# Advanced-Vision-and-Learning-Lab/sparse-view-3dgs-pack

Hardware: AMD Instinct MI355X
Metric: train-step views/s (fwd+bwd) @1M Gaussians 1080p (higher is better)
Workload: dtype f32

## Files before the change

include/gsplat.h:

```cpp
#ifndef GSPLAT_H_INCLUDED
#define GSPLAT_H_INCLUDED

#include <stddef.h>
#include <stdint.h>

#ifdef __cplusplus
extern "C" {
#endif

#define GS_ABI_VERSION 7

#define GS_OK 0
#define GS_E_NULL (-1)
#define GS_E_SHAPE (-2)
#define GS_E_SCRATCH (-3)
#define GS_E_OVERFLOW (-4)
#define GS_E_UNSUPPORTED (-5)

#define GS_TILE_X 16
#define GS_TILE_Y 16
#define GS_NUM_CHANNELS 3

typedef struct GsView {
  int32_t image_height;
  int32_t image_width;
  float tanfovx;
  float tanfovy;
  float scale_modifier;
  int32_t sh_degree;
  int32_t prefiltered;
  int32_t antialiasing;
  int32_t debug;
  int32_t tile_cull;
  const float* bg;
  const float* viewmatrix;
  const float* projmatrix;
  const float* campos;
} GsView;

typedef struct GsGaussians {
  int32_t P;
  int32_t M;
  const float* means3D;
  const float* shs;
  const float* colors_precomp;
  const float* opacities;
  const float* scales;
  const float* rotations;
  const float* cov3D_precomp;
  const float* extra_channel;
  int32_t raw_activations;
  const float* extra_gain;
  const float* shs_rest;
} GsGaussians;

typedef struct GsScratch {
  void* geom;
  size_t geom_bytes;
  void* img;
  size_t img_bytes;
  void* binning;
  size_t binning_bytes;
  int64_t binning_capacity;
  const uint32_t* tile_order_hint;
  const float* tile_depth_limit;
  uint32_t* tile_order_out;
  float* tile_depth_limit_out;
  int32_t binned;
  int32_t defer_tile_order;
  const uint32_t* step_tag;
  const float* tile_depth_limit_slack;
  uint32_t* status_host;
} GsScratch;

typedef struct GsGrads {
  float* dL_dmeans3D;
  float* dL_dmeans2D;
  float* dL_dsh;
  float* dL_dcolors;
  float* dL_dopacity;
  float* dL_dscales;
  float* dL_drotations;
  float* dL_dcov3D;
  float* dL_dextra;
} GsGrads;

int gs_abi_version(void);
const char* gs_build_info(void);
size_t gs_struct_bytes(int32_t which);

int gs_scratch_bytes(int32_t P, int32_t W, int32_t H, int64_t R_capacity, size_t out[3],
                     size_t* backward_workspace_bytes);

int gs_forward_geometry(const GsView* view, const GsGaussians* g, GsScratch* scratch,
                        int32_t* radii, int32_t* num_rendered_host, void* stream);

int gs_forward_render(const GsView* view, const GsGaussians* g, GsScratch* scratch,
                      float* out_color, float* out_invdepth, void* stream);

int gs_forward_bin(const GsView* view, const GsGaussians* g, GsScratch* scratch, uint32_t* status_host, void* stream);

int gs_forward_render_x(const GsView* view, const GsGaussians* g, GsScratch* scratch,
                        float* out_color, float* out_invdepth, float* out_extra, void* stream);

int gs_backward(const GsView* view, const GsGaussians* g, const int32_t* radii,
                const GsScratch* scratch, int64_t num_rendered, const float* dL_dcolor,
                const float* dL_dinvdepth, const GsGrads* grads, void* workspace,
                size_t workspace_bytes, void* stream);

int gs_backward_x(const GsView* view, const GsGaussians* g, const int32_t* radii,
                  const GsScratch* scratch, int64_t num_rendered, const float* dL_dcolor,
                  const float* dL_dinvdepth, const float* dL_dextra_img, const GsGrads* grads,
                  void* workspace, size_t workspace_bytes, void* stream);

int gs_backward_split(const GsView* view, const GsGaussians* g, const int32_t* radii,
                      const GsScratch* scratch, int64_t num_rendered, const float* dL_dcolor,
                      const float* dL_dinvdepth, const GsGrads* grads, float* dL_dsh_rest, void* workspace,
                      size_t workspace_bytes, void* stream);

int gs_forward_render_fsgs(const GsView* view, const GsGaussians* g, GsScratch* scratch,
                           float* out_color, float* out_depth, float* out_alpha, void* stream);
int gs_backward_fsgs(const GsView* view, const GsGaussians* g, const int32_t* radii,
                     const GsScratch* scratch, int64_t num_rendered, const float* dL_dcolor,
                     const float* dL_ddepth, const float* dL_dalpha, const GsGrads* grads,
                     void* workspace, size_t workspace_bytes, void* stream);

int gs_depth_forward(const GsView* view, const GsGaussians* g, GsScratch* scratch, float* out_depth,
                     float* out_alpha, void* stream);
int gs_depth_backward(const GsView* view, const GsGaussians* g, const int32_t* radii,
                      const GsScratch* scratch, int64_t num_rendered, const float* dL_ddepth,
                      const float* dL_dalpha, int grad_flags, float* dL_dmeans3D, float* dL_dmeans2D,
                      float* dL_dopacity, void* workspace, size_t workspace_bytes, void* stream);

#define GS_DEPTH_STEP_ROWS_GIVEN 1
int gs_depth_backward_step(const GsView* view, const GsGaussians* g, const int32_t* radii,
                           const GsScratch* scratch, int64_t num_rendered, const float* dL_ddepth,
                           const float* dL_dalpha, int which, float* param, float* exp_avg, float* exp_avg_sq,
                           float lr, int32_t step, float beta1, float beta2, float eps, int32_t flags,
                           void* workspace, size_t workspace_bytes, void* stream);

int gs_mark_visible(int32_t P, const float* means3D, const float* viewmatrix,
                    const float* projmatrix, uint8_t* present, void* stream);

int gs_region_coop(int32_t form);

int gs_export_geom(const GsScratch* scratch, int32_t P, float* depths, float* means2D ,
                   float* cov3D , float* conic_opacity , float* rgb ,
                   uint8_t* clamped , uint32_t* tiles_touched, uint32_t* point_offsets,
                   void* stream);
int gs_export_binning(const GsScratch* scratch, int64_t num_rendered, uint64_t* keys_sorted,
                      uint32_t* point_list, void* stream);
int gs_export_img(const GsScratch* scratch, int32_t W, int32_t H, float* final_T,
                  uint32_t* n_contrib, uint32_t* ranges , void* stream);

typedef struct GsStepState {
  float* xyz;
  float* features;
  float* opacity;
  float* scaling;
  float* rotation;
  float* m[5];
  float* v[5];
  float lr[6];
  int32_t step[5];
  float beta1, beta2, eps;
  float* max_radii2D;
  float* xyz_gradient_accum;
  float* denom;
  const float* coef_dev;
  const double* rows_override;
  float* grad_out[5];
  float* fail_flag;
  int32_t phase;
  int32_t rows_clean;
  void* phase1_done;
  float* extra;
  float* extra_m;
  float* extra_v;
  float* gain;
  float* gain_m;
  float* gain_v;
  float lr_extra, lr_gain;
  int32_t step_extra, step_gain;
  float* grad_out_extra;
  float* grad_out_gain;
  uint8_t* grad_mask;
  uint8_t* dormant;
  int32_t sparse;
  int32_t reached_split;
  float* grad_out_rest;
} GsStepState;
#define GS_STEP_BLOCK 256
int gs_backward_step(const GsView* view, const GsGaussians* g, const int32_t* radii,
                     const GsScratch* scratch, int64_t num_rendered, const float* dL_dcolor,
                     const float* dL_dinvdepth, const GsStepState* st, void* workspace,
                     size_t workspace_bytes, void* stream);
int gs_backward_step_x(const GsView* view, const GsGaussians* g, const int32_t* radii,
                       const GsScratch* scratch, int64_t num_rendered, const float* dL_dcolor,
                       const float* dL_dinvdepth, const float* dL_dextra_img, const GsStepState* st,
                       void* workspace, size_t workspace_bytes, void* stream);
int gs_backward_step_fsgs(const GsView* view, const GsGaussians* g, const int32_t* radii,
                          const GsScratch* scratch, int64_t num_rendered, const float* dL_dcolor,
                          const float* dL_ddepth, const float* dL_dalpha, const GsStepState* st,
                          void* workspace, size_t workspace_bytes, void* stream);

int gs_step_uninstanced(const GsView* view, const GsGaussians* g, const int32_t* radii,
                        const GsScratch* scratch, const GsStepState* st, void* stream);

int gs_backward_from_rows(const GsView* view, const GsGaussians* g, const int32_t* radii,
                          const GsScratch* scratch, const double* rows, int32_t depth_mode,
                          const GsGrads* grads, void* workspace, size_t workspace_bytes, void* stream);

int gs_export_tile_order(const GsScratch* scratch, int32_t W, int32_t H, uint32_t* out, void* stream);

size_t gs_tile_depth_limit_floats(int32_t W, int32_t H);
int gs_export_tile_stop_depth(const GsScratch* scratch, int32_t W, int32_t H, float* out, void* stream);
#define GS_STATUS_CHECK(tag, num_rendered, overflow, trunc_failed) \
  ((((uint32_t)(tag)) * 2654435761u) ^ (((uint32_t)(num_rendered)) * 40503u) ^ (((uint32_t)(overflow)) << 30) ^ \
   (((uint32_t)(trunc_failed)) << 31) ^ 0x5bd1e995u)
int gs_forward_status(const GsScratch* scratch, uint32_t* out , void* stream);
int gs_forward_tile_order(const GsView* view, const GsScratch* scratch, void* stream);
int gs_debug_blend_stats(const GsScratch* scratch, int32_t P, int32_t W, int32_t H, uint64_t* out, void* stream);
int gs_export_binning_region(const GsScratch* scratch, int32_t W, int32_t H, int64_t num_rendered, uint64_t* keys_sorted,
                             uint32_t* point_list, void* stream);
size_t gs_debug_sort_tmp_bytes(int64_t n_bound);
int gs_debug_sort_pairs(const uint32_t* keys, const uint32_t* vals, const uint32_t* n_dev, int64_t n_bound, int32_t end_bit,
                        int32_t start_buf, int32_t digit_bits, int32_t depth_form, void* tmp, size_t tmp_bytes,
                        uint32_t* keys_out, uint32_t* vals_out, uint32_t* n_kept, uint32_t* digit_totals, void* stream);
int gs_debug_scan_sums(uint32_t* sums, int32_t nb, void* stream);

size_t gs_knn_tmp_bytes(int32_t P);
int gs_knn_mean_dist2(const float* xyz , int32_t P, float* out , void* tmp,
                      size_t tmp_bytes, void* stream);
int gs_knn_mean_dist2_idx(const float* xyz , int32_t P, float* out ,
                          int32_t* nearest , void* tmp, size_t tmp_bytes, void* stream);

size_t gs_grid_encode_tmp_bytes(int64_t B, int32_t D, int32_t L, int32_t C, int64_t n_slots);
int gs_grid_encode_fwd(const float* inputs, int64_t B, int32_t D, const float* embeddings, int64_t n_slots, int32_t C,
                       const int32_t* offsets, int32_t L, float S, int32_t H, int32_t gridtype, int32_t align_corners,
                       int32_t interp, float* outputs, float* dy_dx, void* stream);
int gs_grid_encode_bwd(const float* grad, const float* inputs, int64_t B, int32_t D, int64_t n_slots, int32_t C,
                       const int32_t* offsets, int32_t L, float S, int32_t H, int32_t gridtype, int32_t align_corners,
                       int32_t interp, const float* dy_dx, float* grad_embeddings, float* grad_inputs, void* tmp,
                       size_t tmp_bytes, void* stream);
int gs_sh_encode_fwd(const float* inputs, int64_t B, int32_t degree, float* outputs, void* stream);
int gs_sh_encode_bwd(const float* grad, const float* inputs, int64_t B, int32_t degree, float* grad_inputs, void* stream);

#define GS_DN_GLOBAL 1
#define GS_DN_L1 2
size_t gs_depth_norm_tmp_bytes(int32_t H, int32_t W, int32_t p_local, int32_t p_global);
int gs_depth_norm_fwd(const float* input, const float* target, int32_t H, int32_t W, int32_t p, float margin, int32_t flags,
                      void* tmp, float* loss_out, uint8_t* mask_out , void* stream);
int gs_depth_norm_bwd(const float* input, const float* target, int32_t H, int32_t W, int32_t p, float margin, int32_t flags,
                      const void* tmp, const float* dloss_dev, float* grad_input , void* stream);
int gs_depth_smooth_fwd(const float* depth, const float* img, int32_t C, int32_t H, int32_t W, void* tmp, float* loss_out,
                        void* stream);
int gs_depth_smooth_bwd(const float* depth, const float* img, int32_t C, int32_t H, int32_t W, const void* tmp,
                        const float* dloss_dev, float* grad_depth , void* stream);
int gs_dng_depth_reg_fwd(const float* input, const float* target, int32_t H, int32_t W, int32_t p_local, int32_t p_global,
                         float margin, float w_local, float w_global, float w_smooth, void* tmp, float* loss_out ,
                         uint8_t* mask_local, uint8_t* mask_global, void* stream);
int gs_dng_depth_reg_bwd(const float* input, const float* target, int32_t H, int32_t W, int32_t p_local, int32_t p_global,
                         float margin, float w_local, float w_global, float w_smooth, const void* tmp, const float* dloss_dev,
                         float* grad_input , void* stream);

#define GS_PEARSON_ID 0
#define GS_PEARSON_NEG 1
#define GS_PEARSON_RECIP200 2
#define GS_PEARSON_WRT_R 1
#define GS_PEARSON_BLOCK_ELEMS 4096
#define GS_PEARSON_MAX_BLOCKS 512
size_t gs_pearson_tmp_bytes(int64_t n);
int gs_pearson_fwd(const float* x, const float* t, int64_t n, int32_t form_a, int32_t form_b , void* tmp,
                   float* out , int32_t* branch_out, void* stream);
int gs_pearson_bwd(const float* x, const float* t, int64_t n, int32_t form_a, int32_t form_b, int32_t flags, const void* tmp,
                   const float* dout_dev, float* grad_x , float* grad_t , void* stream);

#define GS_DNG_ENC_X 32
#define GS_DNG_ENC_D 16
#define GS_DNG_HIDDEN 64
#define GS_DNG_GEO 64
#define GS_DNG_HEADS_TILE_ROWS 128
#define GS_DNG_HEADS_MAX_BLOCKS 256
size_t gs_dng_heads_tmp_bytes(int64_t B);
int gs_dng_heads_fwd(const float* enc_x, const float* enc_d, int64_t B, const float* w_s0, const float* w_s1, const float* w_s2,
                     const float* w_c0, const float* w_c1, float* sigma , float* color , int32_t max_blocks,
                     void* stream);
int gs_dng_heads_bwd(const float* enc_x, const float* enc_d, int64_t B, const float* w_s0, const float* w_s1, const float* w_s2,
                     const float* w_c0, const float* w_c1, const float* g_sigma, const float* g_color, float* g_enc_x,
                     float* g_enc_d, float* g_w_s0, float* g_w_s1, float* g_w_s2, float* g_w_c0, float* g_w_c1, void* tmp,
// ... 339 lines not shown
```

sparse-view-3dgs-pack_amd/csrc/gs_api.hip:

```cpp
#include <stdio.h>
#include <stdlib.h>
#include <string.h>
#include <math.h>

#include "gs_common.h"
#include "gs_tilecull.h"
#include "gs_prof.h"

static int check_args(const GsView* v, const GsGaussians* g) {
  if (!v || !g) return GS_E_NULL;
  if (g->P < 0 || v->image_width <= 0 || v->image_height <= 0) return GS_E_SHAPE;
  if (g->P == 0) return GS_OK;
  if (!g->means3D || !g->opacities || !v->viewmatrix || !v->projmatrix || !v->bg) return GS_E_NULL;
  if ((g->shs == nullptr) == (g->colors_precomp == nullptr)) return GS_E_SHAPE;
  const bool has_sr = g->scales != nullptr && g->rotations != nullptr;
  const bool any_sr = g->scales != nullptr || g->rotations != nullptr;
  if ((!has_sr && g->cov3D_precomp == nullptr) || (any_sr && g->cov3D_precomp != nullptr)) return GS_E_SHAPE;
  if (g->shs && (g->M < (v->sh_degree + 1) * (v->sh_degree + 1) || !v->campos)) return GS_E_SHAPE;
  if (v->sh_degree < 0 || v->sh_degree > 3) return GS_E_SHAPE;
  if (g->shs_rest && (!g->shs || g->M < 2)) return GS_E_SHAPE;
  if (v->image_width > 65535 * TILE_X || v->image_height > 65535 * TILE_Y) return GS_E_UNSUPPORTED;
  return GS_OK;
}

static bool reached_marking() {
  static const bool on = [] { const char* e = getenv("GS_REACHED_SPLIT"); return !(e && atoi(e) == 0); }();
  return on;
}
static inline bool step_uses_reached(const GsStepState* st) {
  return st && st->reached_split && !st->rows_override && !st->grad_out[0];
}

static inline void tile_grid(const GsView* v, int& gx, int& gy) {
  gx = (v->image_width + TILE_X - 1) / TILE_X;
  gy = (v->image_height + TILE_Y - 1) / TILE_Y;
}

struct RegionLayout {
  uint32_t* count;
  uint2* bucket;
  uint32_t* point_list;
  uint32_t cap;
  int rg_x, rg_y;
};
static int region_layout(const GsView* v, const GsScratch* sc, RegionLayout& rl) {
  int gx, gy;
  tile_grid(v, gx, gy);
  const size_t T = (size_t)gx * gy, N = (size_t)v->image_width * v->image_height;
  if (!sc->img || !sc->binning) return GS_E_NULL;
  if (sc->img_bytes < img_bytes(N, T)) return GS_E_SCRATCH;
  const int64_t cap = sc->binning_capacity;
  if (cap <= 0 || cap > 0xFFFFFFFFll) return GS_E_SHAPE;
  if (sc->binning_bytes < bin_bytes((size_t)cap, T)) return GS_E_SCRATCH;
  rl.rg_x = (gx + RG_TILES - 1) / RG_TILES;
  rl.rg_y = (gy + RG_TILES - 1) / RG_TILES;
  rl.cap = region_capacity(cap, rl.rg_x * rl.rg_y);
  if (rl.cap == 0) return GS_E_SHAPE;
  ImgView iv = img_view(sc->img, N, T);
  SortBufs bv = sort_view(sc->binning, (size_t)cap);
  rl.count = iv.region_count;
  rl.bucket = reinterpret_cast<uint2*>(bv.keys[0]);
  rl.point_list = bv.vals[0];
  return GS_OK;
}

extern "C" {

int gs_abi_version(void) { return GS_ABI_VERSION; }

size_t gs_struct_bytes(int32_t which) {
  switch (which) {
    case 0: return sizeof(GsView);
    case 1: return sizeof(GsGaussians);
    case 2: return sizeof(GsScratch);
    case 3: return sizeof(GsGrads);
    case 4: return sizeof(GsStepState);
    case 5: return sizeof(GsLgdwtParams);
    case 6: return sizeof(GsAdamSeg);
    default: return 0;
  }
}

const char* gs_build_info(void) {
  return "libgsplat_hip gfx950 | hipcc " __VERSION__
         " | preprocess/knn: -ffp-contract=off, blend: fast contract | radix 8-bit LSD | tile 16x16, wave64 8x8 quadrants";
}

int gs_scratch_bytes(int32_t P, int32_t W, int32_t H, int64_t R_capacity, size_t out[3], size_t* bwd_ws) {
  if (!out) return GS_E_NULL;
  if (P < 0 || W <= 0 || H <= 0 || R_capacity < 0) return GS_E_SHAPE;
  const size_t T = (size_t)((W + TILE_X - 1) / TILE_X) * ((H + TILE_Y - 1) / TILE_Y);
  out[0] = geom_bytes((size_t)P);
  out[1] = img_bytes((size_t)W * H, T);
  out[2] = bin_bytes((size_t)R_capacity, T);
  if (bwd_ws) *bwd_ws = bwd_workspace_bytes((size_t)P);
  return GS_OK;
}

int gs_forward_geometry(const GsView* v, const GsGaussians* g, GsScratch* sc, int32_t* radii,
                        int32_t* num_rendered_host, void* stream) {
  int rc = check_args(v, g);
  if (rc) return rc;
  if (!sc || !sc->geom) return GS_E_NULL;
  sc->binned = 0;
  hipStream_t s = (hipStream_t)stream;
  const int P = g->P;
  if (sc->geom_bytes < geom_bytes((size_t)P)) return GS_E_SCRATCH;
  GeomView gv = geom_view(sc->geom, (size_t)P);
  if (P == 0) {
    GS_HIP_CHECK(hipMemsetAsync(gv.hdr, 0, sizeof(GeomHeader), s));
    if (num_rendered_host) GS_HIP_CHECK(hipMemcpyAsync(num_rendered_host, &gv.hdr->num_rendered, 4, hipMemcpyDeviceToHost, s));
    return GS_OK;
  }
  if (!radii) return GS_E_NULL;
  PreprocessArgs a;
  a.P = P;
  a.D = v->sh_degree;
  a.M = g->M;
  a.means3D = g->means3D;
  a.scales = g->scales;
  a.scale_modifier = v->scale_modifier;
  a.rotations = g->rotations;
  a.opacities = g->opacities;
  a.raw_activations = g->raw_activations;
  a.shs = g->shs;
  a.shs_rest = g->shs_rest;
  a.cov3D_precomp = g->cov3D_precomp;
  a.colors_precomp = g->colors_precomp;
  a.viewmatrix = v->viewmatrix;
  a.projmatrix = v->projmatrix;
  a.campos = v->campos;
  a.W = v->image_width;
  a.H = v->image_height;
  a.focal_y = v->image_height / (2.0f * v->tanfovy);
  a.focal_x = v->image_width / (2.0f * v->tanfovx);
  a.tan_fovx = v->tanfovx;
  a.tan_fovy = v->tanfovy;
  a.radii = radii;
  tile_grid(v, a.grid_x, a.grid_y);
  a.antialiasing = v->antialiasing;
  a.extra_channel = g->extra_channel;
  a.extra_gain = g->extra_gain;
  a.tile_cull = v->tile_cull;
  a.tile_depth_limit = v->tile_cull ? sc->tile_depth_limit : nullptr;
  a.region_count = nullptr;
  a.region_bucket = nullptr;
  a.region_cap = 0;
  a.rg_x = a.rg_y = 0;
  if (v->tile_cull == 2) {
    RegionLayout rl;
    rc = region_layout(v, sc, rl);
    if (rc) return rc;
    a.region_count = rl.count;
    a.region_bucket = rl.bucket;
    a.region_cap = rl.cap;
    a.rg_x = rl.rg_x;
    a.rg_y = rl.rg_y;
    launch_region_prepare(gv, rl.count, rl.rg_x * rl.rg_y, (uint32_t)P, s);
    GS_LAUNCH_CHECK(s, v->debug);
  }
  {
    GS_PROF(ST_PREPROCESS_FWD, s);
    launch_preprocess_fwd(a, gv, s);
  }
  GS_LAUNCH_CHECK(s, v->debug);
  if (v->tile_cull != 2) {
    GS_PROF(ST_SCAN, s);
    launch_scan_block_sums(gv, P, s);
  }
  GS_LAUNCH_CHECK(s, v->debug);
  if (num_rendered_host)
    GS_HIP_CHECK(hipMemcpyAsync(num_rendered_host, &gv.hdr->num_rendered, 4, hipMemcpyDeviceToHost, s));
  return GS_OK;
}

int gs_forward_render(const GsView* v, const GsGaussians* g, GsScratch* sc, float* out_color, float* out_invdepth,
                      void* stream) {
  return gs_forward_render_x(v, g, sc, out_color, out_invdepth, nullptr, stream);
}

static int forward_bin_stage(const GsView* v, const GsScratch* sc, const GeomView& gv, const ImgView& iv, const SortBufs& bv, int P,
                             int gx, int gy, hipStream_t s) {
  int rc;
  const int64_t cap = sc->binning_capacity;
  const size_t T = (size_t)gx * gy;
  if (v->tile_cull == 2) {
    RegionLayout rl;
    rc = region_layout(v, sc, rl);
    if (rc) return rc;
    GS_PROF(ST_SORT, s);
    rc = launch_region_bin(gv, rl.count, rl.bucket, rl.cap, rl.rg_x, rl.rg_y, gx, gy, sc->tile_depth_limit, iv.ranges, rl.point_list,
                           cap, s);
    if (rc) return rc;
    GS_LAUNCH_CHECK(s, v->debug);
    return GS_OK;
  }
  launch_bin_prepare(gv, cap, iv.ranges, (int)T, s);
  GS_LAUNCH_CHECK(s, v->debug);
  if (cap > 0) {
    {
      GS_PROF(ST_SORT_DEPTH, s);
      rc = launch_radix_sort(gv.gsort, &gv.hdr->P, P, 32, 0, gv.depth_keys, s, v->debug, &gv.hdr->n_ordered);
      if (rc) return rc;
    }
    const TileBinView tb = tilebin_view((char*)sc->binning + sort_bytes((size_t)cap), (size_t)cap, T);
    rc = launch_tile_binning(gv, bv, tb, P, cap, gx, gy, v->tile_cull, sc->tile_depth_limit, iv.ranges, (v->debug & 2) ? 1 : 0, s,
                             v->debug & 1);
    if (rc) return rc;
  }
  GS_LAUNCH_CHECK(s, v->debug);
  return GS_OK;
}

static int forward_render_impl(const GsView* v, const GsGaussians* g, GsScratch* sc, float* out_color, float* out_invdepth,
                               float* out_extra, int fsgs, void* stream);

int gs_forward_bin(const GsView* v, const GsGaussians* g, GsScratch* sc, uint32_t* status_host, void* stream) {
  int rc = check_args(v, g);
  if (rc) return rc;
  if (!sc || !sc->geom || !sc->img) return GS_E_NULL;
  hipStream_t s = (hipStream_t)stream;
  const int P = g->P, W = v->image_width, H = v->image_height;
  int gx, gy;
  tile_grid(v, gx, gy);
  const size_t T = (size_t)gx * gy, N = (size_t)W * H;
  if (sc->img_bytes < img_bytes(N, T)) return GS_E_SCRATCH;
  if (P > 0) {
    if (sc->geom_bytes < geom_bytes((size_t)P)) return GS_E_SCRATCH;
    const int64_t cap = sc->binning_capacity;
    if (cap < 0) return GS_E_SHAPE;
    if (cap > 0 && (!sc->binning || sc->binning_bytes < bin_bytes((size_t)cap, T))) return GS_E_SCRATCH;
    if (cap > 0xFFFFFFFFll) return GS_E_UNSUPPORTED;
    GeomView gv = geom_view(sc->geom, (size_t)P);
    ImgView iv = img_view(sc->img, N, T);
    SortBufs bv = sort_view(sc->binning, (size_t)cap);
    rc = forward_bin_stage(v, sc, gv, iv, bv, P, gx, gy, s);
    if (rc) return rc;
  }
  sc->binned = 1;
  if (status_host) GS_HIP_CHECK(hipMemcpyAsync(status_host, sc->geom, 16, hipMemcpyDeviceToHost, s));
  return GS_OK;
}

int gs_forward_render_x(const GsView* v, const GsGaussians* g, GsScratch* sc, float* out_color, float* out_invdepth,
                        float* out_extra, void* stream) {
  if (out_extra && g && !g->extra_channel) return GS_E_NULL;
  return forward_render_impl(v, g, sc, out_color, out_invdepth, out_extra, 0, stream);
}

int gs_forward_render_fsgs(const GsView* v, const GsGaussians* g, GsScratch* sc, float* out_color, float* out_depth,
                           float* out_alpha, void* stream) {
  if (!out_depth || !out_alpha) return GS_E_NULL;
  if (v && v->antialiasing) return GS_E_UNSUPPORTED;
  return forward_render_impl(v, g, sc, out_color, out_depth, out_alpha, 1, stream);
}
// ... 771 lines not shown
```

sparse-view-3dgs-pack_amd/csrc/gs_common.h:

```cpp
#pragma once
#include <hip/hip_runtime.h>
#include <stdint.h>

#include "../../include/gsplat.h"

#define GS_BLOCK 256
#define TILE_X GS_TILE_X
#define TILE_Y GS_TILE_Y

struct GeomHeader {
  uint32_t num_rendered;
  uint32_t overflow;
  uint32_t trunc_failed;
  uint32_t zero;
  uint32_t P;
  uint32_t sort_n;
  uint32_t n_ordered;
  uint32_t region_mode;
  uint32_t step_tag;
  uint32_t pad[55];
};
#define HDR_SIDE_CURSOR 1
#define HDR_LIMITED 2
#define HDR_REACHED 3
// ... 138 lines not shown
  v.region_ranges = (uint2*)p; p += gs_align(8 * T);
  v.chunk_first = (uint32_t*)p; p += gs_align(4 * (T + 1));
  v.chunk_desc = (uint4*)p; p += gs_align(16 * mc);
  v.chunk_counts = (uint32_t*)p; p += gs_align(64 * mc);
  v.tile_start = (uint32_t*)p;
  v.max_chunks = (uint32_t)mc;
  return v;
}
static inline __host__ __device__ size_t bin_bytes(size_t cap, size_t T) { return sort_bytes(cap) + tilebin_bytes(cap, T); }

enum { GR_MX = 0, GR_MY, GR_CXX, GR_CXY, GR_CYY, GR_OP, GR_CR, GR_CG, GR_CB, GR_ID, GR_EXTRA, GR_N, GR_STRIDE = 16 };
typedef double gs_row_t;
#define GR_ROW_BYTES (GR_STRIDE * sizeof(gs_row_t))
enum { GC_MX = 0, GC_MY, GC_DMX, GC_DMY, GC_DMZ, GC_DOP, GC_C0, GC_R = GC_C0 + 7, GC_G, GC_B, GC_EXTRA, GC_STRIDE = 20 };
#define GC_REC_BYTES (GC_STRIDE * sizeof(float))
static inline __host__ __device__ size_t bwd_workspace_bytes(size_t P) {
  return gs_align(P * GR_ROW_BYTES) + gs_align(P * GC_REC_BYTES) + gs_align(4 * ((P + GS_BLOCK - 1) / GS_BLOCK + 4));
}

static inline uint32_t gs_higher_msb(uint32_t n) {
  uint32_t msb = sizeof(n) * 4;
  uint32_t step = msb;
  while (step > 1) {
    step /= 2;
    if (n >> msb)
      msb += step;
    else
      msb -= step;
  }
  if (n >> msb) msb++;
  return msb;
}

#define GS_HIP_CHECK(expr)                 \
  do {                                     \
    hipError_t _e = (expr);                \
    if (_e != hipSuccess) return (int)_e;  \
  } while (0)

static inline int gs_after_launch(hipStream_t s, int debug) {
  hipError_t e = hipGetLastError();
  if (e != hipSuccess) return (int)e;
  if (debug) {
    e = hipStreamSynchronize(s);
    if (e != hipSuccess) return (int)e;
  }
  return 0;
}
#define GS_LAUNCH_CHECK(stream, debug)             \
  do {                                             \
    int _rc = gs_after_launch((stream), (debug));  \
    if (_rc) return _rc;                           \
  } while (0)

struct PreprocessArgs {
  int P, D, M;
  const float* means3D;
  const float* scales;
  float scale_modifier;
  const float* rotations;
  const float* opacities;
  const float* shs;
  const float* shs_rest;
  const float* cov3D_precomp;
  const float* colors_precomp;
  const float* viewmatrix;
  const float* projmatrix;
  const float* campos;
  int W, H;
  float focal_x, focal_y, tan_fovx, tan_fovy;
  int* radii;
  int grid_x, grid_y;
  int antialiasing;
  const float* extra_channel;
  const float* extra_gain;
  int tile_cull;
  const float* tile_depth_limit;
  int raw_activations;
  uint32_t* region_count;
  uint2* region_bucket;
  uint32_t region_cap;
  int rg_x, rg_y;
};
int launch_preprocess_fwd(const PreprocessArgs& a, const GeomView& g, hipStream_t s);
int launch_scan_block_sums(const GeomView& g, int P, hipStream_t s);
int launch_mark_visible(int P, const float* means3D, const float* viewmatrix, uint8_t* present, hipStream_t s);

int launch_bin_prepare(const GeomView& g, int64_t capacity, uint2* ranges, int T, hipStream_t s);
int launch_radix_sort(const SortBufs& b, const uint32_t* n_dev, int64_t n_host_bound, int end_bit, int start_buf,
                      const uint32_t* first_keys, hipStream_t s, int debug, uint32_t* n_kept = nullptr, int digit_bits = 8);
int launch_scan_sums(uint32_t* sums, int nb, hipStream_t s);
int launch_tile_binning(const GeomView& g, const SortBufs& bv, const TileBinView& tb, int P, int64_t capacity, int grid_x, int grid_y,
                        int tile_cull, const float* tile_depth_limit, uint2* ranges, int force_rowwise, hipStream_t s, int debug);

#define RG_TILES 4
#define RG_MAX_ENTRIES 16384
static inline __host__ __device__ uint32_t region_capacity(int64_t capacity, int regions) {
  const int64_t c = regions > 0 ? capacity / regions : 0;
  return (uint32_t)(c > RG_MAX_ENTRIES ? RG_MAX_ENTRIES : (c < 0 ? 0 : c));
}
int launch_region_prepare(const GeomView& g, uint32_t* region_count, int regions, uint32_t P, hipStream_t s);
int launch_region_bin(const GeomView& g, const uint32_t* region_count, const uint2* region_bucket, uint32_t region_cap, int rg_x,
                      int rg_y, int grid_x, int grid_y, const float* tile_depth_limit, uint2* ranges, uint32_t* point_list,
                      int64_t capacity, hipStream_t s);
int launch_export_keys_region(const uint2* ranges, const uint32_t* point_list, const Splat* splat, int T, uint64_t* keys_sorted,
                              hipStream_t s);


int launch_render_fwd_wave(const uint2* ranges, const uint32_t* point_list, int W, int H, int grid_x, int grid_y,
                           const Splat* splat, const float* bg, float* final_T, uint32_t* n_contrib, uint32_t* tile_work,
                           const uint32_t* order_hint, const float* depth_limit, float* stop_depth, uint32_t* trunc_failed,
                           float* out_color, float* out_invdepth, float* out_extra, int fsgs, int cull, hipStream_t s,
                           uint8_t* reached = nullptr, uint32_t* reached_flag = nullptr);
int launch_export_stop_depth(const float* stop_depth, float* out, int grid_x, int grid_y, hipStream_t s);
int launch_tile_order(const uint32_t* tile_work, uint32_t* tile_order, int T, uint32_t* order_out, const float* stop_depth,
                      float* limit_out, int grid_x, int grid_y, const GeomHeader* hdr, hipStream_t s,
                      const float* slack_dev = nullptr, uint32_t* status_host = nullptr, const uint32_t* step_tag = nullptr);
int launch_zero_rows(gs_row_t* rows, size_t P, const uint32_t* tiles_touched, hipStream_t s);
int launch_render_bwd_wave(const uint2* ranges, const uint32_t* point_list, int W, int H, int grid_x, int grid_y,
                           const Splat* splat, const float* bg, const float* final_T, const uint32_t* n_contrib,
                           const uint32_t* tile_work, const uint32_t* tile_order, const float* dL_dpix,
                           const float* dL_dinvdepth, const float* dL_dextra, gs_row_t* grad_rows, int fsgs, hipStream_t s);

int launch_depth_fwd(const uint2* ranges, const uint32_t* point_list, int W, int H, int grid_x, int grid_y, const Splat* splat,
                     float* final_T, uint32_t* n_contrib, uint32_t* tile_work, float* stop_depth, float* out_depth,
                     float* out_alpha, int cull, hipStream_t s);
int launch_depth_bwd(const uint2* ranges, const uint32_t* point_list, int W, int H, int grid_x, int grid_y, const Splat* splat,
                     const float* final_T, const uint32_t* n_contrib, const uint32_t* tile_work, const uint32_t* tile_order,
                     const float* dL_ddepth, const float* dL_dalpha, gs_row_t* grad_rows, int grad_flags, hipStream_t s);
struct DepthPointArgs {
  int P;
  const float* means3D;
  const int* radii;
  const float* scales;
  const float* rotations;
  float scale_modifier;
  const float* cov3D;
  const float* viewmatrix;
  const float* projmatrix;
  float focal_x, focal_y, tan_fovx, tan_fovy;
  int skip_uninstanced;
  const uint32_t* tiles_touched;
  const gs_row_t* grad_rows;
  float* dL_dmeans3D;
  float* dL_dmeans2D;
  float* dL_dopacity;
};
int launch_depth_point_bwd(const DepthPointArgs& a, int grad_flags, hipStream_t s);
struct DepthStepArgs {
  float* param;
  float* exp_avg;
  float* exp_avg_sq;
  const float* activated;
  float lr_bc1, inv_sqrt_bc2, b1, b2, eps;
};
int launch_depth_point_step(const DepthPointArgs& a, const DepthStepArgs& st, int which, hipStream_t s);

int launch_blend_stats(const uint2* ranges, const uint32_t* point_list, int W, int H, int grid_x, int grid_y, const Splat* splat,
                       const uint32_t* n_contrib, const uint32_t* tile_work, unsigned long long* out, hipStream_t s);

struct PreprocessBwdArgs {
  int P, D, M;
  const float* means3D;
  const int* radii;
  const float* shs;
  const float* shs_rest;
  const float* scales;
  const float* rotations;
  const float* opacities;
  const float* colors_precomp;
  float scale_modifier;
  const float* cov3D;
  const float* viewmatrix;
  const float* projmatrix;
  const float* campos;
  float focal_x, focal_y, tan_fovx, tan_fovy;
  int antialiasing;
  int has_invdepth;
  int has_extra;
  const float* extra_raw;
  const float* extra_gain;
  float* gain_partials;
  int raw_activations;
  int skip_uninstanced;
// ... 29 lines not shown
```

sparse-view-3dgs-pack_amd/csrc/gs_preprocess.hip:

```cpp
#include "gs_common.h"
#include "gs_tilecull.h"
#include "gs_math.h"

template <typename SH>
GS_DEV V3 color_from_sh(int deg, V3 pos, V3 campos, const SH& sh, uint32_t& clamped) {
  V3 dir = pos - campos;
  dir = dir / length3(dir);
  V3 result = SH_C0 * sh(0);
  if (deg > 0) {
    float x = dir.x, y = dir.y, z = dir.z;
    result = result - SH_C1 * y * sh(1) + SH_C1 * z * sh(2) - SH_C1 * x * sh(3);
    if (deg > 1) {
      float xx = x * x, yy = y * y, zz = z * z;
      float xy = x * y, yz = y * z, xz = x * z;
      result = result + SH_C2_0 * xy * sh(4) + SH_C2_1 * yz * sh(5) + SH_C2_2 * (2.0f * zz - xx - yy) * sh(6) +
               SH_C2_3 * xz * sh(7) + SH_C2_4 * (xx - yy) * sh(8);
      if (deg > 2) {
        result = result + SH_C3_0 * y * (3.0f * xx - yy) * sh(9) + SH_C3_1 * xy * z * sh(10) +
                 SH_C3_2 * y * (4.0f * zz - xx - yy) * sh(11) + SH_C3_3 * z * (2.0f * zz - 3.0f * xx - 3.0f * yy) * sh(12) +
                 SH_C3_4 * x * (4.0f * zz - xx - yy) * sh(13) + SH_C3_5 * z * (xx - yy) * sh(14) +
                 SH_C3_6 * x * (xx - 3.0f * yy) * sh(15);
      }
    }
  }
  result.x += 0.5f;
  result.y += 0.5f;
  result.z += 0.5f;
  clamped = (result.x < 0 ? 1u : 0u) | (result.y < 0 ? 2u : 0u) | (result.z < 0 ? 4u : 0u);
  return {fmaxf(result.x, 0.0f), fmaxf(result.y, 0.0f), fmaxf(result.z, 0.0f)};
}

struct ShRegs {
  float f[48];
  __device__ __forceinline__ V3 operator()(int k) const { return {f[3 * k], f[3 * k + 1], f[3 * k + 2]}; }
};
struct ShMem {
  const float* p;
  __device__ __forceinline__ V3 operator()(int k) const { return {p[3 * k], p[3 * k + 1], p[3 * k + 2]}; }
};
struct ShMemSplit {
  const float *dc, *rest;
  __device__ __forceinline__ V3 operator()(int k) const {
    const float* p = k == 0 ? dc : rest + 3 * (k - 1);
    return {p[0], p[1], p[2]};
  }
};

#ifndef GS_LIMIT_TILES_IN_LDS
#define GS_LIMIT_TILES_IN_LDS 0
#endif
#define GS_LIMIT_LDS_MAX_FLOATS (GS_LIMIT_TILES_IN_LDS ? 10240 : 4096)
extern __shared__ float s_limit[];
static inline size_t preprocess_limit_lds_floats(const PreprocessArgs& a) {
  if (!a.tile_depth_limit) return 0;
  const size_t T = (size_t)a.grid_x * a.grid_y, all = depth_limit_floats((uint32_t)a.grid_x, (uint32_t)a.grid_y);
  const size_t want = GS_LIMIT_TILES_IN_LDS ? all : all - T;
  return want <= GS_LIMIT_LDS_MAX_FLOATS ? want : 0;
}

#ifndef GS_REGION_COOP_DEFAULT
#define GS_REGION_COOP_DEFAULT 1
#endif
#define GS_COOP_PAIRS 2
struct CoopWave {
  uint32_t pref[64];
  uint32_t dbits[64];
  uint32_t r0[64];
  uint32_t nrx[64];
  uint32_t tiles[64];
};

template <bool COOP>
__global__ void __launch_bounds__(GS_BLOCK) preprocess_fwd_kernel(PreprocessArgs a, GeomView g, int lds_floats) {
  const int idx = blockIdx.x * GS_BLOCK + threadIdx.x;
  uint32_t tiles = 0, entries = TB_ENTRIES_UNKNOWN;
  const int T = a.grid_x * a.grid_y;
  int p0 = 0, p1 = 0, p2 = 0, p3 = 0, n_pend = 0;
  uint32_t s0 = 0xFFFFFFFFu, s1 = 0xFFFFFFFFu, s2 = 0xFFFFFFFFu, s3 = 0xFFFFFFFFu, dbits = 0;
  auto bump = [&]() {
    if (n_pend > 0) s0 = atomicAdd(&a.region_count[(size_t)p0 * RG_COUNT_STRIDE], 1u);
    if (n_pend > 1) s1 = atomicAdd(&a.region_count[(size_t)p1 * RG_COUNT_STRIDE], 1u);
    if (n_pend > 2) s2 = atomicAdd(&a.region_count[(size_t)p2 * RG_COUNT_STRIDE], 1u);
    if (n_pend > 3) s3 = atomicAdd(&a.region_count[(size_t)p3 * RG_COUNT_STRIDE], 1u);
    n_pend = 0;
  };
  auto collect = [&]() {
    const uint2 entry = make_uint2(dbits, (uint32_t)idx);
    if (s0 < a.region_cap) a.region_bucket[(size_t)p0 * a.region_cap + s0] = entry;
    if (s1 < a.region_cap) a.region_bucket[(size_t)p1 * a.region_cap + s1] = entry;
    if (s2 < a.region_cap) a.region_bucket[(size_t)p2 * a.region_cap + s2] = entry;
    if (s3 < a.region_cap) a.region_bucket[(size_t)p3 * a.region_cap + s3] = entry;
    s0 = s1 = s2 = s3 = 0xFFFFFFFFu;
  };
  const int lidx = min(idx, a.P - 1);
  typedef const __attribute__((address_space(4))) float* GsConstFloatPtr;
  float vm[16], pm[16], cam[3];
  {
    const GsConstFloatPtr vmp = (GsConstFloatPtr)(uintptr_t)a.viewmatrix, pmp = (GsConstFloatPtr)(uintptr_t)a.projmatrix;
    const GsConstFloatPtr cp = (GsConstFloatPtr)(uintptr_t)a.campos;
#pragma unroll
    for (int k = 0; k < 16; k++) { vm[k] = vmp[k]; pm[k] = pmp[k]; }
    cam[0] = cp[0]; cam[1] = cp[1]; cam[2] = cp[2];
  }
  const bool own_cov = a.cov3D_precomp == nullptr;
  const float* sc_p = own_cov ? a.scales + 3 * (size_t)lidx : a.cov3D_precomp + 6 * (size_t)lidx;
  const float* rq_p = own_cov ? a.rotations + 4 * (size_t)lidx : a.cov3D_precomp + 6 * (size_t)lidx;
  float op_in = a.opacities[lidx];
  V3 p_orig = {a.means3D[3 * (size_t)lidx], a.means3D[3 * (size_t)lidx + 1], a.means3D[3 * (size_t)lidx + 2]};
  V3 sc_in = {sc_p[0], sc_p[1], sc_p[2]};
  V4 rq_in = {rq_p[0], rq_p[1], rq_p[2], rq_p[3]};
  if (lds_floats) {
    const float* src = a.tile_depth_limit + (GS_LIMIT_TILES_IN_LDS ? 0 : T);
    for (int i = threadIdx.x; i < lds_floats; i += GS_BLOCK) s_limit[i] = src[i];
    __syncthreads();
  }
  asm volatile("" : "+v"(op_in), "+v"(sc_in.x), "+v"(sc_in.y), "+v"(sc_in.z), "+v"(rq_in.x), "+v"(rq_in.y), "+v"(rq_in.z),
               "+v"(rq_in.w));
  const GsLdsFloatPtr lds_seg = (GsLdsFloatPtr)s_limit + (GS_LIMIT_TILES_IN_LDS ? T : 0);
  if (idx == 0) {
    g.hdr->pad[HDR_LIMITED] = a.tile_depth_limit ? 1u : 0u;
    g.hdr->pad[HDR_REACHED] = 0u;
  }
  const int segs_x = (int)depth_limit_segs_x((uint32_t)a.grid_x);
  auto region_bound = [&](int rx, int ry) {
    float bound = -__builtin_inff();
#pragma unroll
    for (int k = 0; k < RG_TILES; k++) {
      const int ty = min(ry * RG_TILES + k, a.grid_y - 1);
      const float v = lds_floats ? lds_seg[ty * segs_x + rx] : a.tile_depth_limit[(size_t)T + ty * segs_x + rx];
      bound = fmaxf(bound, v);
    }
    return bound;
  };
  Splat sp;
  sp.x = sp.y = sp.depth = sp.invdepth = 0.f;
  sp.cxx = sp.cxy = sp.cyy = sp.opacity = 0.f;
  sp.r = sp.g = sp.b = 0.f;
  sp.extra = 0.f;
  int radius_out = 0;
  sp.rect_min = sp.rect_max = sp.tiles = sp.clamped = 0;
  float cov3D[6] = {0, 0, 0, 0, 0, 0};
  bool write_cov = false;
  bool reached = false;
  uint32_t big_n = 0, big_r0 = 0, big_nrx = 0;

  auto finish = [&]() {
    sp.clamped |= (tiles ? entries : 0u) << 16;
    if (!(a.tile_depth_limit && tiles == 0)) {
      if (a.colors_precomp == nullptr) {
        V3 campos = {cam[0], cam[1], cam[2]};
        V3 rgb;
        uint32_t cl = 0;
        if (a.M == 16 && a.shs_rest) {
          ShRegs sh;
          const float* dc = a.shs + (size_t)idx * 3;
          const float* rest = a.shs_rest + (size_t)idx * 45;
          const int nfl = 3 * (a.D + 1) * (a.D + 1) - 3;
          sh.f[0] = dc[0]; sh.f[1] = dc[1]; sh.f[2] = dc[2];
#pragma unroll
          for (int k = 0; k < 45; k++) sh.f[3 + k] = k < nfl ? rest[k] : 0.f;
          bump();
          rgb = color_from_sh(a.D, p_orig, campos, sh, cl);
        } else if (a.M == 16) {
          ShRegs sh;
          const float4* src = reinterpret_cast<const float4*>(a.shs + (size_t)idx * 48);
          const int nvec = a.D == 0 ? 1 : (a.D == 1 ? 3 : (a.D == 2 ? 7 : 12));
#pragma unroll
          for (int k = 0; k < 12; k++) {
            if (k < nvec) {
              float4 v = src[k];
              sh.f[4 * k] = v.x; sh.f[4 * k + 1] = v.y; sh.f[4 * k + 2] = v.z; sh.f[4 * k + 3] = v.w;
            } else {
              sh.f[4 * k] = sh.f[4 * k + 1] = sh.f[4 * k + 2] = sh.f[4 * k + 3] = 0.f;
            }
          }
          bump();
          rgb = color_from_sh(a.D, p_orig, campos, sh, cl);
        } else if (a.shs_rest) {
          bump();
          ShMemSplit sh{a.shs + (size_t)idx * 3, a.shs_rest + (size_t)idx * (a.M - 1) * 3};
          rgb = color_from_sh(a.D, p_orig, campos, sh, cl);
        } else {
          bump();
          ShMem sh{a.shs + (size_t)idx * a.M * 3};
          rgb = color_from_sh(a.D, p_orig, campos, sh, cl);
        }
        sp.r = rgb.x; sp.g = rgb.y; sp.b = rgb.z;
        sp.clamped |= cl;
      } else {
        bump();
        sp.r = a.colors_precomp[3 * idx];
        sp.g = a.colors_precomp[3 * idx + 1];
        sp.b = a.colors_precomp[3 * idx + 2];
      }
    }
    sp.tiles = tiles;
  };

  bool write_record = true;
  auto store_record = [&](int half) {
    float4* dst = reinterpret_cast<float4*>(&g.splat[idx]);
    const float4* srcv = reinterpret_cast<const float4*>(&sp);
// ... 256 lines not shown
        coop_collect();
      }
      coop_bump(base);
    }
    if (idx < a.P) store_geometry();
    if (reached) finish();
    if (idx < a.P) {
      if (write_record) store_record(1);
      collect();
    }
  } else if (idx < a.P) {
    store_geometry();
    if (write_record) store_record(1);
    collect();
    if (a.tile_cull != 2) g.depth_keys[idx] = tiles ? __float_as_uint(sp.depth) : 0xFFFFFFFFu;
  }
  if constexpr (COOP) coop_collect();
  __shared__ uint32_t red[GS_BLOCK / 64];
  uint32_t v = tiles;
#pragma unroll
  for (int off = 32; off >= 1; off >>= 1) v += __shfl_down(v, off, 64);
  if ((threadIdx.x & 63) == 0) red[threadIdx.x >> 6] = v;
  __syncthreads();
  if (threadIdx.x == 0) g.block_sums[blockIdx.x] = red[0] + red[1] + red[2] + red[3];
}

__global__ void __launch_bounds__(1024) scan_block_sums_kernel(GeomView g, int nb, uint32_t P) {
  __shared__ uint32_t wsum[16];
  __shared__ uint32_t carry_s;
  const int tid = threadIdx.x, lane = tid & 63, wid = tid >> 6;
  if (tid == 0) carry_s = 0;
  __syncthreads();
  for (int base = 0; base < nb; base += 1024) {
    int i = base + tid;
    uint32_t v = (i < nb) ? g.block_sums[i] : 0u;
    uint32_t inc = v;
#pragma unroll
    for (int off = 1; off < 64; off <<= 1) {
      uint32_t t = __shfl_up(inc, off, 64);
      if (lane >= off) inc += t;
    }
    if (lane == 63) wsum[wid] = inc;
    __syncthreads();
    uint32_t woff = 0;
    for (int w = 0; w < wid; w++) woff += wsum[w];
    uint32_t carry = carry_s;
    if (i < nb) g.block_sums[i] = carry + woff + inc - v;
    __syncthreads();
    if (tid == 1023) carry_s = carry + woff + inc;
    __syncthreads();
  }
  if (tid == 0) {
    g.block_sums[nb] = carry_s;
    g.hdr->num_rendered = carry_s;
    g.hdr->overflow = 0;
    g.hdr->P = P;
    g.hdr->region_mode = 0;
    g.hdr->pad[HDR_SIDE_CURSOR] = 0;
  }
}

__global__ void __launch_bounds__(GS_BLOCK) mark_visible_kernel(int P, const float* means3D, const float* vm,
                                                                uint8_t* present) {
  const int idx = blockIdx.x * GS_BLOCK + threadIdx.x;
  if (idx >= P) return;
  V3 p = {means3D[3 * idx], means3D[3 * idx + 1], means3D[3 * idx + 2]};
  V3 pv = xform4x3(p, vm);
  present[idx] = !(pv.z <= 0.2f);
}

static int g_region_coop = -1;
static int region_coop_form() {
  if (g_region_coop < 0) {
    const char* e = getenv("GS_REGION_COOP");
    g_region_coop = e ? (atoi(e) != 0 ? 1 : 0) : GS_REGION_COOP_DEFAULT;
  }
  return g_region_coop;
}
extern "C" int gs_region_coop(int32_t form) {
  if (form >= 0) g_region_coop = form ? 1 : 0;
  return region_coop_form();
}

int launch_preprocess_fwd(const PreprocessArgs& a, const GeomView& g, hipStream_t s) {
  const int nb = (a.P + GS_BLOCK - 1) / GS_BLOCK;
  const size_t lds = preprocess_limit_lds_floats(a);
  const bool coop = a.tile_cull == 2 && region_coop_form() && a.rg_x <= 0xFFFF && a.rg_y <= 0xFFFF &&
                    (long long)a.rg_x * a.rg_y <= (1ll << 26);
  if (coop)
    hipLaunchKernelGGL(preprocess_fwd_kernel<true>, dim3(nb), dim3(GS_BLOCK), 4 * lds, s, a, g, (int)lds);
  else
    hipLaunchKernelGGL(preprocess_fwd_kernel<false>, dim3(nb), dim3(GS_BLOCK), 4 * lds, s, a, g, (int)lds);
  return 0;
}
int launch_scan_block_sums(const GeomView& g, int P, hipStream_t s) {
  const int nb = (P + GS_BLOCK - 1) / GS_BLOCK;
  hipLaunchKernelGGL(scan_block_sums_kernel, dim3(1), dim3(1024), 0, s, g, nb, (uint32_t)P);
  return 0;
}
int launch_mark_visible(int P, const float* means3D, const float* viewmatrix, uint8_t* present, hipStream_t s) {
  hipLaunchKernelGGL(mark_visible_kernel, dim3((P + GS_BLOCK - 1) / GS_BLOCK), dim3(GS_BLOCK), 0, s, P, means3D,
                     viewmatrix, present);
  return 0;
}
```

sparse-view-3dgs-pack_amd/csrc/gs_regionbin.hip:

```cpp
#include "gs_common.h"
#include "gs_tilecull.h"

#define RB_THREADS 1024
#define RB_WAVES (RB_THREADS / 64)
#define RB_TILES (RG_TILES * RG_TILES)

__global__ void __launch_bounds__(GS_BLOCK) region_prepare_kernel(GeomHeader* hdr, uint32_t* __restrict__ region_count,
                                                                   int regions, uint32_t P) {
  const int i = blockIdx.x * GS_BLOCK + threadIdx.x;
  if (i < regions) region_count[(size_t)i * RG_COUNT_STRIDE] = 0u;
  if (i == 0) {
    hdr->num_rendered = 0u;
    hdr->overflow = 0u;
    hdr->trunc_failed = 0u;
    hdr->zero = 0u;
    hdr->P = P;
    hdr->sort_n = 0u;
    hdr->n_ordered = 0u;
    hdr->region_mode = 1u;
    hdr->pad[HDR_SIDE_CURSOR] = 0u;
  }
}

__global__ void __launch_bounds__(RB_THREADS) region_bin_kernel(GeomHeader* hdr, const Splat* __restrict__ splat,
                                                                 const uint32_t* __restrict__ region_count,
                                                                 const uint2* __restrict__ region_bucket, uint32_t region_cap,
                                                                 int rg_x, int grid_x, int grid_y,
                                                                 const float* __restrict__ depth_limit,
                                                                 uint2* __restrict__ ranges, uint32_t* __restrict__ point_list,
                                                                 uint32_t capacity, uint32_t n_pad_max) {
  extern __shared__ unsigned long long s_key[];
  __shared__ uint32_t s_wcnt[RB_WAVES][RB_TILES];
  __shared__ uint32_t s_off[RB_TILES + 1];
  __shared__ uint32_t s_base;
  __shared__ float s_lim[RB_TILES];
  const int tid = threadIdx.x, lane = tid & 63, wid = tid >> 6;
  const int r = blockIdx.x, rx = r % rg_x, ry = r / rg_x;
  const uint32_t cnt_raw = region_count[(size_t)r * RG_COUNT_STRIDE];
  const uint32_t n = min(min(cnt_raw, region_cap), n_pad_max);
  if (tid == 0) {
    atomicMax(&hdr->zero, cnt_raw);
    if (cnt_raw > n) hdr->overflow = 1u;
  }
  if (tid < RB_TILES) {
    const int ty = ry * RG_TILES + (tid >> 2), tx = rx * RG_TILES + (tid & 3);
    s_lim[tid] = (depth_limit && ty < grid_y && tx < grid_x) ? depth_limit[ty * grid_x + tx] : __builtin_inff();
  }
  uint32_t n_pad = 64;
  while (n_pad < n) n_pad <<= 1;
  const uint2* bucket = region_bucket + (size_t)r * region_cap;
  for (uint32_t i = tid; i < n_pad; i += RB_THREADS) {
    unsigned long long k = ~0ull;
    if (i < n) {
      const uint2 e = bucket[i];
      k = ((unsigned long long)e.x << 32) | (unsigned long long)e.y;
    }
    s_key[i] = k;
  }
  __syncthreads();
  auto step = [&](uint32_t k, uint32_t j) {
    for (uint32_t i = tid; i < (n_pad >> 1); i += RB_THREADS) {
      const uint32_t lo = ((i & ~(j - 1u)) << 1) | (i & (j - 1u));
      const uint32_t hi = lo | j;
      const unsigned long long a = s_key[lo], b = s_key[hi];
      const bool up = (lo & k) == 0u;
      if ((a > b) == up) {
        s_key[lo] = b;
        s_key[hi] = a;
      }
    }
  };
  for (uint32_t k = 2; k <= n_pad; k <<= 1) {
    uint32_t j = k >> 1;
    for (; j > 64; j >>= 1) {
      step(k, j);
      __syncthreads();
    }
    for (; j > 0; j >>= 1) {
      step(k, j);
      __builtin_amdgcn_fence(__ATOMIC_RELEASE, "wavefront");
      __builtin_amdgcn_wave_barrier();
      __builtin_amdgcn_fence(__ATOMIC_ACQUIRE, "wavefront");
    }
    if (k >= 128u || k == n_pad) __syncthreads();
  }
  for (uint32_t e = tid; e < n; e += RB_THREADS) {
    const uint32_t id = (uint32_t)s_key[e];
    const float4* rec = reinterpret_cast<const float4*>(&splat[id]);
    const float4 ra = rec[0], rc = rec[1];
    const uint4 tail = reinterpret_cast<const uint4*>(rec)[3];
    const TileCull tc = tilecull_setup(1, ra.x, ra.y, rc.x, rc.y, rc.z, rc.w);
    const uint32_t rminx = tail.x & 0xFFFFu, rminy = tail.x >> 16, rmaxx = tail.y & 0xFFFFu, rmaxy = tail.y >> 16;
    uint32_t mask = 0;
#pragma unroll
// ... 13 lines not shown
    }
    s_key[e] = ((unsigned long long)mask << 32) | (unsigned long long)id;
  }
  __syncthreads();
  const uint32_t per_wave = ((n + RB_WAVES * 64 - 1) / (RB_WAVES * 64)) * 64;
  const uint32_t w_lo = min((uint32_t)wid * per_wave, n), w_hi = min(w_lo + per_wave, n);
  uint32_t my_cnt = 0;
  for (uint32_t e0 = w_lo; e0 < w_hi; e0 += 64) {
    const uint32_t e = e0 + lane;
    const uint32_t m = e < w_hi ? (uint32_t)(s_key[e] >> 32) : 0u;
#pragma unroll
    for (uint32_t t = 0; t < RB_TILES; t++) {
      const uint32_t c = (uint32_t)__popcll(__ballot((m >> t) & 1u));
      if (lane == (int)t) my_cnt += c;
    }
  }
  if (lane < RB_TILES) s_wcnt[wid][lane] = my_cnt;
  __syncthreads();
  if (tid < RB_TILES) {
    uint32_t run = 0;
#pragma unroll
    for (int w = 0; w < RB_WAVES; w++) {
      const uint32_t c = s_wcnt[w][tid];
      s_wcnt[w][tid] = run;
      run += c;
    }
    s_off[tid + 1] = run;
  }
  __syncthreads();
  if (tid == 0) {
    uint32_t run = 0;
    s_off[0] = 0;
    for (int t = 0; t < RB_TILES; t++) {
      const uint32_t c = s_off[t + 1];
      s_off[t] = run;
      run += c;
    }
    s_off[RB_TILES] = run;
    uint32_t base = 0xFFFFFFFFu;
    if (run) {
      const uint32_t at = atomicAdd(&hdr->num_rendered, run);
      if ((unsigned long long)at + run <= (unsigned long long)capacity) base = at;
      else hdr->overflow = 1u;
    } else {
      base = 0u;
    }
    s_base = base;
  }
  __syncthreads();
  const uint32_t base = s_base;
  if (tid < RB_TILES) {
    const int ty = ry * RG_TILES + (tid >> 2), tx = rx * RG_TILES + (tid & 3);
    if (ty < grid_y && tx < grid_x) {
      const uint32_t b = base + s_off[tid], c = s_off[tid + 1] - s_off[tid];
      ranges[ty * grid_x + tx] = (base == 0xFFFFFFFFu || c == 0u) ? make_uint2(0u, 0u) : make_uint2(b, b + c);
    }
  }
  if (base == 0xFFFFFFFFu) return;
  uint32_t run = 0;
  const unsigned long long lt_mask = lane == 0 ? 0ull : (~0ull >> (64 - lane));
  for (uint32_t e0 = w_lo; e0 < w_hi; e0 += 64) {
    const uint32_t e = e0 + lane;
    const unsigned long long k = e < w_hi ? s_key[e] : 0ull;
    const uint32_t m = (uint32_t)(k >> 32), id = (uint32_t)k;
#pragma unroll
    for (uint32_t t = 0; t < RB_TILES; t++) {
      const unsigned long long b = __ballot((m >> t) & 1u);
      const uint32_t before = (uint32_t)__shfl((int)run, (int)t, 64);
      if ((m >> t) & 1u) point_list[base + s_off[t] + s_wcnt[wid][t] + before + (uint32_t)__popcll(b & lt_mask)] = id;
      if (lane == (int)t) run += (uint32_t)__popcll(b);
    }
  }
}

__global__ void __launch_bounds__(GS_BLOCK) export_keys_region_kernel(const uint2* __restrict__ ranges,
                                                                      const uint32_t* __restrict__ point_list,
                                                                      const Splat* __restrict__ splat,
                                                                      uint64_t* __restrict__ keys_sorted) {
  const uint2 r = ranges[blockIdx.x];
  for (uint32_t i = r.x + threadIdx.x; i < r.y; i += GS_BLOCK)
    keys_sorted[i] = ((uint64_t)blockIdx.x << 32) | (uint64_t)__float_as_uint(splat[point_list[i]].depth);
}

int launch_region_prepare(const GeomView& g, uint32_t* region_count, int regions, uint32_t P, hipStream_t s) {
  hipLaunchKernelGGL(region_prepare_kernel, dim3((regions + GS_BLOCK - 1) / GS_BLOCK > 0 ? (regions + GS_BLOCK - 1) / GS_BLOCK : 1),
                     dim3(GS_BLOCK), 0, s, g.hdr, region_count, regions, P);
  return 0;
}

int launch_region_bin(const GeomView& g, const uint32_t* region_count, const uint2* region_bucket, uint32_t region_cap, int rg_x,
                      int rg_y, int grid_x, int grid_y, const float* tile_depth_limit, uint2* ranges, uint32_t* point_list,
                      int64_t capacity, hipStream_t s) {
  uint32_t n_pad = 1024;
  while (n_pad < region_cap && n_pad < RG_MAX_ENTRIES) n_pad <<= 1;
  const size_t lds = (size_t)n_pad * sizeof(unsigned long long);
  static_assert(RG_MAX_ENTRIES * sizeof(unsigned long long) <= 160 * 1024, "a region's sort must fit gfx950's 160 KB of LDS");
  static size_t lds_allowed[64] = {};
  int dev = 0;
  if (hipGetDevice(&dev) != hipSuccess || dev < 0 || dev >= 64) dev = -1;
  if (dev < 0 || lds > lds_allowed[dev]) {
    hipError_t e = hipFuncSetAttribute((const void*)region_bin_kernel, hipFuncAttributeMaxDynamicSharedMemorySize, (int)lds);
    if (e != hipSuccess) return (int)e;
    if (dev >= 0) lds_allowed[dev] = lds;
  }
  const uint32_t cap32 = capacity > 0xFFFFFFFFll ? 0xFFFFFFFFu : (capacity < 0 ? 0u : (uint32_t)capacity);
  hipLaunchKernelGGL(region_bin_kernel, dim3(rg_x * rg_y), dim3(RB_THREADS), lds, s, g.hdr, g.splat, region_count, region_bucket,
                     region_cap, rg_x, grid_x, grid_y, tile_depth_limit, ranges, point_list, cap32, n_pad);
  const hipError_t le = hipGetLastError();
  return le == hipSuccess ? 0 : (int)le;
}

int launch_export_keys_region(const uint2* ranges, const uint32_t* point_list, const Splat* splat, int T, uint64_t* keys_sorted,
                              hipStream_t s) {
  hipLaunchKernelGGL(export_keys_region_kernel, dim3(T), dim3(GS_BLOCK), 0, s, ranges, point_list, splat, keys_sorted);
  return 0;
}
```

sparse-view-3dgs-pack_amd/gsplat_amd/capi.py:

```python
import ctypes as C
import os

c_f_p = C.c_void_p


class GsView(C.Structure):
    _fields_ = [
        ("image_height", C.c_int32),
        ("image_width", C.c_int32),
        ("tanfovx", C.c_float),
        ("tanfovy", C.c_float),
        ("scale_modifier", C.c_float),
        ("sh_degree", C.c_int32),
        ("prefiltered", C.c_int32),
        ("antialiasing", C.c_int32),
        ("debug", C.c_int32),
        ("tile_cull", C.c_int32),
        ("bg", C.c_void_p),
        ("viewmatrix", C.c_void_p),
        ("projmatrix", C.c_void_p),
        ("campos", C.c_void_p),
    ]


class GsGaussians(C.Structure):
    _fields_ = [
        ("P", C.c_int32),
        ("M", C.c_int32),
        ("means3D", C.c_void_p),
        ("shs", C.c_void_p),
        ("colors_precomp", C.c_void_p),
        ("opacities", C.c_void_p),
        ("scales", C.c_void_p),
        ("rotations", C.c_void_p),
        ("cov3D_precomp", C.c_void_p),
        ("extra_channel", C.c_void_p),
        ("raw_activations", C.c_int32),
        ("extra_gain", C.c_void_p),
        ("shs_rest", C.c_void_p),
    ]


class GsScratch(C.Structure):
    _fields_ = [
        ("geom", C.c_void_p),
        ("geom_bytes", C.c_size_t),
        ("img", C.c_void_p),
        ("img_bytes", C.c_size_t),
        ("binning", C.c_void_p),
        ("binning_bytes", C.c_size_t),
        ("binning_capacity", C.c_int64),
        ("tile_order_hint", C.c_void_p),
        ("tile_depth_limit", C.c_void_p),
        ("tile_order_out", C.c_void_p),
        ("tile_depth_limit_out", C.c_void_p),
        ("binned", C.c_int32),
        ("defer_tile_order", C.c_int32),
        ("step_tag", C.c_void_p),
        ("tile_depth_limit_slack", C.c_void_p),
        ("status_host", C.c_void_p),
    ]


class GsGrads(C.Structure):
    _fields_ = [
        ("dL_dmeans3D", C.c_void_p),
        ("dL_dmeans2D", C.c_void_p),
        ("dL_dsh", C.c_void_p),
        ("dL_dcolors", C.c_void_p),
        ("dL_dopacity", C.c_void_p),
        ("dL_dscales", C.c_void_p),
        ("dL_drotations", C.c_void_p),
        ("dL_dcov3D", C.c_void_p),
        ("dL_dextra", C.c_void_p),
    ]


class GsLgdwtParams(C.Structure):
    _fields_ = [("lambda_dssim", C.c_float), ("n_pix", C.c_float), ("n_band1", C.c_float), ("n_band2", C.c_float),
                ("dwt_w", C.c_float * 8), ("patch_w", C.c_float * 3), ("patch_weight", C.c_float),
                ("patch_elems_per_sel", C.c_float), ("dwt_enable", C.c_int32), ("patch_enable", C.c_int32),
                ("reset_sums", C.c_int32), ("custom_base", C.c_int32), ("w_l1", C.c_float), ("w_ssim", C.c_float)]


class GsAdamSeg(C.Structure):
    _fields_ = [("begin", C.c_int64), ("end", C.c_int64), ("lr_a", C.c_float), ("lr_b", C.c_float),
                ("period", C.c_int32), ("split", C.c_int32), ("step", C.c_int32), ("row_width", C.c_int32)]


class GsAdamTensor(C.Structure):
    _fields_ = [("param", C.c_void_p), ("grad", C.c_void_p), ("exp_avg", C.c_void_p), ("exp_avg_sq", C.c_void_p),
                ("n", C.c_int64), ("row_width", C.c_int32), ("step", C.c_int32), ("lr", C.c_float), ("pad", C.c_int32)]


ADAM_NO_BIAS_CORRECTION = 1
DEPTH_STEP_ROWS_GIVEN = 1
ADAM_MAX_TENSORS = 8


class GsStepState(C.Structure):
    _fields_ = [("xyz", C.c_void_p), ("features", C.c_void_p), ("opacity", C.c_void_p), ("scaling", C.c_void_p),
                ("rotation", C.c_void_p), ("m", C.c_void_p * 5), ("v", C.c_void_p * 5), ("lr", C.c_float * 6),
                ("step", C.c_int32 * 5), ("beta1", C.c_float), ("beta2", C.c_float), ("eps", C.c_float),
                ("max_radii2D", C.c_void_p), ("xyz_gradient_accum", C.c_void_p), ("denom", C.c_void_p),
                ("coef_dev", C.c_void_p), ("rows_override", C.c_void_p), ("grad_out", C.c_void_p * 5),
                ("fail_flag", C.c_void_p), ("phase", C.c_int32), ("rows_clean", C.c_int32),
                ("phase1_done", C.c_void_p),
                ("extra", C.c_void_p), ("extra_m", C.c_void_p), ("extra_v", C.c_void_p), ("gain", C.c_void_p),
                ("gain_m", C.c_void_p), ("gain_v", C.c_void_p), ("lr_extra", C.c_float), ("lr_gain", C.c_float),
                ("step_extra", C.c_int32), ("step_gain", C.c_int32), ("grad_out_extra", C.c_void_p),
                ("grad_out_gain", C.c_void_p), ("grad_mask", C.c_void_p), ("dormant", C.c_void_p), ("sparse", C.c_int32),
                ("reached_split", C.c_int32),
                ("grad_out_rest", C.c_void_p)]


_P = C.c_void_p
_I32 = C.c_int32
_I64 = C.c_int64
_F = C.c_float
_SZ = C.c_size_t

PROTOTYPES = {
    "abi_version": (C.c_int, []),
    "struct_bytes": (C.c_size_t, [C.c_int32]),
    "build_info": (C.c_char_p, []),
    "scratch_bytes": (C.c_int, [_I32, _I32, _I32, _I64, C.POINTER(_SZ), C.POINTER(_SZ)]),
    "forward_geometry": (C.c_int, [C.POINTER(GsView), C.POINTER(GsGaussians), C.POINTER(GsScratch), _P, _P, _P]),
    "forward_render": (C.c_int, [C.POINTER(GsView), C.POINTER(GsGaussians), C.POINTER(GsScratch), _P, _P, _P]),
    "backward": (C.c_int, [C.POINTER(GsView), C.POINTER(GsGaussians), _P, C.POINTER(GsScratch), _I64, _P, _P,
                           C.POINTER(GsGrads), _P, _SZ, _P]),
    "forward_render_x": (C.c_int, [C.POINTER(GsView), C.POINTER(GsGaussians), C.POINTER(GsScratch), _P, _P, _P, _P]),
    "backward_split": (C.c_int, [C.POINTER(GsView), C.POINTER(GsGaussians), _P, C.POINTER(GsScratch), _I64, _P, _P,
                                 C.POINTER(GsGrads), _P, _P, _SZ, _P]),
    "backward_x": (C.c_int, [C.POINTER(GsView), C.POINTER(GsGaussians), _P, C.POINTER(GsScratch), _I64, _P, _P, _P,
                             C.POINTER(GsGrads), _P, _SZ, _P]),
    "forward_render_fsgs": (C.c_int, [C.POINTER(GsView), C.POINTER(GsGaussians), C.POINTER(GsScratch), _P, _P, _P, _P]),
    "backward_fsgs": (C.c_int, [C.POINTER(GsView), C.POINTER(GsGaussians), _P, C.POINTER(GsScratch), _I64, _P, _P, _P,
                                C.POINTER(GsGrads), _P, _SZ, _P]),
    "depth_forward": (C.c_int, [C.POINTER(GsView), C.POINTER(GsGaussians), C.POINTER(GsScratch), _P, _P, _P]),
    "depth_backward": (C.c_int, [C.POINTER(GsView), C.POINTER(GsGaussians), _P, C.POINTER(GsScratch), _I64, _P, _P, C.c_int,
                                 _P, _P, _P, _P, _SZ, _P]),
    "depth_backward_step": (C.c_int, [C.POINTER(GsView), C.POINTER(GsGaussians), _P, C.POINTER(GsScratch), _I64, _P, _P, C.c_int,
                                      _P, _P, _P, _F, _I32, _F, _F, _F, _I32, _P, _SZ, _P]),
    "step_uninstanced": (C.c_int, [C.POINTER(GsView), C.POINTER(GsGaussians), _P, C.POINTER(GsScratch),
                                   C.POINTER(GsStepState), _P]),
    "backward_step": (C.c_int, [C.POINTER(GsView), C.POINTER(GsGaussians), _P, C.POINTER(GsScratch), _I64, _P, _P,
                                C.POINTER(GsStepState), _P, _SZ, _P]),
    "backward_step_x": (C.c_int, [C.POINTER(GsView), C.POINTER(GsGaussians), _P, C.POINTER(GsScratch), _I64, _P, _P, _P,
                                  C.POINTER(GsStepState), _P, _SZ, _P]),
    "backward_step_fsgs": (C.c_int, [C.POINTER(GsView), C.POINTER(GsGaussians), _P, C.POINTER(GsScratch), _I64, _P, _P, _P,
                                     C.POINTER(GsStepState), _P, _SZ, _P]),
    "backward_from_rows": (C.c_int, [C.POINTER(GsView), C.POINTER(GsGaussians), _P, C.POINTER(GsScratch), _P, _I32,
                                     C.POINTER(GsGrads), _P, _SZ, _P]),
    "mark_visible": (C.c_int, [_I32, _P, _P, _P, _P, _P]),
    "region_coop": (C.c_int, [_I32]),
    "export_geom": (C.c_int, [C.POINTER(GsScratch), _I32, _P, _P, _P, _P, _P, _P, _P, _P, _P]),
    "export_binning": (C.c_int, [C.POINTER(GsScratch), _I64, _P, _P, _P]),
    "export_img": (C.c_int, [C.POINTER(GsScratch), _I32, _I32, _P, _P, _P, _P]),
    "export_tile_order": (C.c_int, [C.POINTER(GsScratch), _I32, _I32, _P, _P]),
    "export_tile_stop_depth": (C.c_int, [C.POINTER(GsScratch), _I32, _I32, _P, _P]),
    "forward_status": (C.c_int, [C.POINTER(GsScratch), _P, _P]),
    "forward_tile_order": (C.c_int, [C.POINTER(GsView), C.POINTER(GsScratch), _P]),
    "forward_bin": (C.c_int, [C.POINTER(GsView), C.POINTER(GsGaussians), C.POINTER(GsScratch), _P, _P]),
    "export_binning_region": (C.c_int, [C.POINTER(GsScratch), _I32, _I32, _I64, _P, _P, _P]),
    "debug_blend_stats": (C.c_int, [C.POINTER(GsScratch), _I32, _I32, _I32, _P, _P]),
    "debug_sort_tmp_bytes": (_SZ, [_I64]),
    "debug_sort_pairs": (C.c_int, [_P, _P, _P, _I64, _I32, _I32, _I32, _I32, _P, _SZ, _P, _P, _P, _P, _P]),
    "debug_scan_sums": (C.c_int, [_P, _I32, _P]),
    "tile_depth_limit_floats": (C.c_size_t, [_I32, _I32]),
    "knn_tmp_bytes": (_SZ, [_I32]),
    "knn_mean_dist2": (C.c_int, [_P, _I32, _P, _P, _SZ, _P]),
    "knn_mean_dist2_idx": (C.c_int, [_P, _I32, _P, _P, _P, _SZ, _P]),
    "grid_encode_tmp_bytes": (_SZ, [_I64, _I32, _I32, _I32, _I64]),
    "grid_encode_fwd": (C.c_int, [_P, _I64, _I32, _P, _I64, _I32, _P, _I32, _F, _I32, _I32, _I32, _I32, _P, _P, _P]),
    "grid_encode_bwd": (C.c_int, [_P, _P, _I64, _I32, _I64, _I32, _P, _I32, _F, _I32, _I32, _I32, _I32, _P, _P, _P, _P,
                                  _SZ, _P]),
    "sh_encode_fwd": (C.c_int, [_P, _I64, _I32, _P, _P]),
    "sh_encode_bwd": (C.c_int, [_P, _P, _I64, _I32, _P, _P]),
    "depth_norm_tmp_bytes": (_SZ, [_I32, _I32, _I32, _I32]),
    "depth_norm_fwd": (C.c_int, [_P, _P, _I32, _I32, _I32, _F, _I32, _P, _P, _P, _P]),
    "depth_norm_bwd": (C.c_int, [_P, _P, _I32, _I32, _I32, _F, _I32, _P, _P, _P, _P]),
    "depth_smooth_fwd": (C.c_int, [_P, _P, _I32, _I32, _I32, _P, _P, _P]),
    "depth_smooth_bwd": (C.c_int, [_P, _P, _I32, _I32, _I32, _P, _P, _P, _P]),
    "dng_depth_reg_fwd": (C.c_int, [_P, _P, _I32, _I32, _I32, _I32, _F, _F, _F, _F, _P, _P, _P, _P, _P]),
    "dng_depth_reg_bwd": (C.c_int, [_P, _P, _I32, _I32, _I32, _I32, _F, _F, _F, _F, _P, _P, _P, _P]),
    "pearson_tmp_bytes": (_SZ, [_I64]),
    "pearson_fwd": (C.c_int, [_P, _P, _I64, _I32, _I32, _P, _P, _P, _P]),
    "pearson_bwd": (C.c_int, [_P, _P, _I64, _I32, _I32, _I32, _P, _P, _P, _P, _P]),
    "dng_heads_tmp_bytes": (_SZ, [_I64]),
    "dng_heads_fwd": (C.c_int, [_P, _P, _I64, _P, _P, _P, _P, _P, _P, _P, _I32, _P]),
    "dng_heads_bwd": (C.c_int, [_P, _P, _I64, _P, _P, _P, _P, _P, _P, _P, _P, _P, _P, _P, _P, _P, _P, _P, _SZ, _I32, _P]),
    "dng_reg_tmp_bytes": (_SZ, [_I64]),
    "dng_reg_fwd": (C.c_int, [_P, _P, _I64, C.c_double, C.c_double, C.c_double, _I32, _I32, _P, _P, _P]),
    "dng_reg_bwd": (C.c_int, [_P, _P, _I64, _I32, _P, _P, _P, _P, _P, _P]),
    "view_dirs_fwd": (C.c_int, [_P, _P, _I64, _P, _P]),
    "view_dirs_bwd": (C.c_int, [_P, _P, _I64, _P, _P, _P]),
    "near_mask": (C.c_int, [_P, _I64, _P, _I32, _F, _P, _P]),
    "dtu_mask": (C.c_int, [_P, _I32, _I32, _F, _I32, _P, _P, _P, _P]),
    "masked_tmp_bytes": (_SZ, [_I64]),
    "masked_fill_fwd": (C.c_int, [_P, _P, _I64, _P, _P, _P, _P]),
    "masked_fill_bwd": (C.c_int, [_P, _P, _I64, _P, _P]),
    "alpha_penalty_fwd": (C.c_int, [_P, _P, _I64, _P, _P, _P]),
    "alpha_penalty_bwd": (C.c_int, [_P, _P, _I64, _P, _P, _P, _P]),
    "dng_colour_rule": (C.c_int, [_P, _P, _P, _I64, _I32, _F, _F, _I32, _I32, _F, _F, _I32, _F, _P, _P]),
    "blender_tmp_bytes": (_SZ, [_I64]),
    "blender_target": (C.c_int, [_P, _P, _I32, _I32, _F, _P, _P, _P, _P, _P]),
    "dng_white_rule": (C.c_int, [_P, _P, _P, _I64, _F, _F, _P, _P]),
    "dng_white_rule_sh": (C.c_int, [_P, _P, _P, _I32, _I32, _P, _P, _P, _I64, _F, _F, _P, _P, _P]),
    "l1_fwd": (C.c_int, [_P, _P, _I64, _P, _P]),
    "l1_bwd": (C.c_int, [_P, _P, _I64, _F, _P, _I32, _P]),
    "dwt_haar_fwd": (C.c_int, [_P, _I32, _I32, _I32, _P, _P, _P, _P, _P]),
    "dwt_haar_bwd": (C.c_int, [_P, _P, _P, _P, _I32, _I32, _I32, _P, _P]),
    "dwt2_l1_fwd": (C.c_int, [_P, _P, _I32, _I32, _I32, _P, _P]),
    "dwt2_l1_bwd": (C.c_int, [_P, _P, _I32, _I32, _I32, _P, _P, _I32, _P]),
    "elf_map": (C.c_int, [_P, _I32, _I32, _I32, _P, _P, _P]),
    "patch_means": (C.c_int, [_P, _I32, _I32, _I32, _P, _P]),
    "patch_dwt_fwd": (C.c_int, [_P, _P, _I32, _I32, _I32, _I32, _P, _P, _P]),
    "patch_dwt_bwd": (C.c_int, [_P, _P, _I32, _I32, _I32, _I32, _P, _P, _P, _I32, _P]),
    "ssim_fwd": (C.c_int, [_P, _P, _I32, _I32, _I32, _I32, _F, _F, _P, _P, _P, _P, _P]),
    "ssim_bwd": (C.c_int, [_P, _P, _I32, _I32, _I32, _I32, _F, _F, _P, _P, _P, _P, _P, _P]),
    "dwt_partials_count": (C.c_int64, [_I32, _I32, _I32]),
    "l1_dwt2_patch_fwd_clamp_p": (C.c_int, [_P, _P, _I32, _I32, _I32, _I32, _P, _P, _P, _P]),
    "l1_partials_count": (C.c_int64, [_I64]),
    "l1_fwd_p": (C.c_int, [_P, _P, _I64, _P, _P]),
    "depth_l1_partials_count": (C.c_int64, [_I64]),
    "depth_l1": (C.c_int, [_P, _P, _P, _I64, _P, _F, _P, _P, _P]),
    "lgdwt_combine_pp": (C.c_int, [_P, _P, _I64, _P, _I64, _P, _I64, _P, C.POINTER(GsLgdwtParams), _P, _P]),
    "l1_bwd_dev": (C.c_int, [_P, _P, _I64, _P, _P, _I32, _P]),
    "l1_dwt2_fwd": (C.c_int, [_P, _P, _I32, _I32, _I32, _P, _P, _P]),
    "l1_dwt2_fwd_clamp": (C.c_int, [_P, _P, _I32, _I32, _I32, _P, _P, _P, _P]),
    "l1_dwt2_patch_fwd_clamp": (C.c_int, [_P, _P, _I32, _I32, _I32, _I32, _P, _P, _P, _P, _P, _P]),
    "l1_dwt2_patch_bwd": (C.c_int, [_P, _P, _I32, _I32, _I32, _I32, _P, _P, _P, _P, _P, _I32, _P]),
    "l1_dwt2_bwd": (C.c_int, [_P, _P, _I32, _I32, _I32, _P, _P, _P, _I32, _P]),
    "ssim_fwd_sum": (C.c_int, [_P, _P, _I32, _I32, _I32, _I32, _F, _F, _P, _P, _P, _P, _P]),
    "ssim_bwd_uniform": (C.c_int, [_P, _P, _I32, _I32, _I32, _I32, _P, _P, _P, _P, _P, _I32, _P, _P]),
    "lgdwt_combine": (C.c_int, [_P, _P, C.POINTER(GsLgdwtParams), _P, _P]),
    "lgdwt_combine_p": (C.c_int, [_P, _P, _I64, _P, C.POINTER(GsLgdwtParams), _P, _P]),
    "ssim_partials_count": (C.c_int64, [_I32, _I32, _I32, _I32]),
    "ssim_fwd_partials": (C.c_int, [_P, _P, _I32, _I32, _I32, _I32, _F, _F, _P, _P, _P, _P, _P]),
    "lgdwt_fused_fwd": (C.c_int, [_P, _P, _I32, _I32, _I32, _F, _F, _I32, _P, _P, _P, _P, _P, _P, _P]),
    "lgdwt_fused_bwd": (C.c_int, [_P, _P, _I32, _I32, _I32, _I32, _I32, _P, _P, _P, _P, _P, _P, _P]),
    "adam_step": (C.c_int, [_P, _P, _P, _P, _I64, C.POINTER(GsAdamSeg), _I32, _F, _F, _F, _I32, _P]),
    "adam_step_gated": (C.c_int, [_P, _P, _P, _P, _I64, C.POINTER(GsAdamSeg), _I32, _F, _F, _F, _I32, _P, _P]),
    "adam_step_masked": (C.c_int, [_P, _P, _P, _P, _I64, C.POINTER(GsAdamSeg), _I32, _F, _F, _F, _I32, _P, _P, _P]),
    "adam_step_tensors": (C.c_int, [C.POINTER(GsAdamTensor), _I32, _I64, _F, _F, _F, _I32, _P, _P]),
    "activations_fwd": (C.c_int, [_P, _P, _P, _I32, _P, _P, _P, _P]),
    "activations_bwd": (C.c_int, [_P, _P, _P, _I32, _P, _P, _P, _P, _P, _P, _P]),
    "densify_stats": (C.c_int, [_P, _P, _I32, _P, _P, _P, _P]),
    "densify_tmp_bytes": (_SZ, [_I32]),
    "densify_plan": (C.c_int, [_P, _P, _P, _P, _I32, _I32, _F, _F, _F, _F, _F, _I32, _P, _SZ, _P]),
    "densify_emit": (C.c_int, [_P, _SZ, _P, _P, _P, _P, _I32, _I32, _I32, _I32, _I32, _I32, _I32, _P, _P, _P]),
    "morton_codes": (C.c_int, [_P, _I64, _P, _P, _P, _P]),
    "densify_gather": (C.c_int, [_P, _P, _P, _I32, _P, _P, _P, _I32, _P, _P, _P, _I32, C.POINTER(C.c_int32), _I32, _I32, _F, _P]),
    "densify_plan_gated": (C.c_int, [_P, _P, _P, _P, _I32, _I32, _F, _F, _F, _F, _F, _I32, _F, _P, _SZ, _P]),
    "prune_tmp_bytes": (_SZ, [_I32]),
    "prune_plan": (C.c_int, [_P, _I32, _P, _SZ, _P]),
    "prune_emit": (C.c_int, [_P, _SZ, _P, _P, _I32, _I32, _P, _P, _P, _P, _P, _P, _P, _P, _P]),
    "densify_fsgs_tmp_bytes": (_SZ, [_I32]),
    "densify_fsgs_plan": (C.c_int, [_P, _P, _P, _P, _P, _I32, _I32, _F, _F, _F, _F, _F, _F, _I32, _P, _SZ, _P, _P]),
    "densify_fsgs_merge": (C.c_int, [_P, _SZ, _P, _I32, _F, _I32, _P]),
    "densify_fsgs_emit": (C.c_int, [_P, _SZ, _P, _P, _P, _P, _I32, _I32, _I32, _I32, _I32, _I32, _I32, _P, _P, _P]),
    "densify_fsgs_prox_plan": (C.c_int, [_P, _SZ, _I32, _P, _I32, _P, _P, _F, _I32, _P, _SZ, _P]),
    "densify_fsgs_final": (C.c_int, [_P, _SZ, _P, _P, _P, _I32, _I32, _I32, _I32, _I32, _P, _P, _P, _P, _P, _P]),
    "densify_fsgs_gather": (C.c_int, [_P, _P, _P, _P, _I32, _P, _P, _P, _I32, _P, _P, _P, _I32, C.POINTER(C.c_int32), _I32, _I32, _I32,
                                      _I32, _F, _P]),
    "profile_enable": (C.c_int, [_I32]),
    "profile_only": (C.c_int, [_I32]),
    "profile_reset": (C.c_int, []),
    "profile_stage_count": (C.c_int, []),
    "rows_pack": (C.c_int, [_P, _I32, _I32, C.POINTER(C.c_int32), _P, _P, _I32, _P, _P]),
    "rows_unpack": (C.c_int, [_P, _I32, _I32, C.POINTER(C.c_int32), _P, _P, _I32, _P, _P]),
    "export_row_mask": (C.c_int, [C.POINTER(GsScratch), _I32, _P, _P]),
    "profile_stage_name": (C.c_char_p, [_I32]),
    "profile_read": (C.c_int, [C.POINTER(C.c_double), C.POINTER(_I64), _I32]),
    "image_stage_partials_count": (C.c_int64, [_I32, _I32]),
    "image_stage_fwd": (C.c_int, [_P, _P, _P, _I32, _I32, _P, _P]),
    "image_stage_bwd": (C.c_int, [_P, _P, _P, _P, _I32, _I32, _P, _P, _P]),
    "exposure_adam": (C.c_int, [_P, _I64, _I32, _P, _P, _P, _P, _I32, _F, C.c_double, C.c_double, _F, _I32, _P, _P]),
    "eval_partials_count": (C.c_int64, [_I32, _I32, _I32]),
    "eval_tmp_bytes": (_SZ, [_I32, _I32, _I32]),
    "eval_metrics": (C.c_int, [_P, _P, _P, _I32, _I32, _I32, _I32, _F, _F, _P, _SZ, _P, _P, _P]),
    "resize_tmp_bytes": (_SZ, [_I32, _I32, _I32, _I32, _I32]),
    "resize_bicubic_u8": (C.c_int, [_P, _I32, _I32, _I32, _I32, _I32, _P, _P, _I32, _P, _P, _I32, _P, _SZ, _P, _P, _P]),
    "eval_ssim_sk_tmp_bytes": (_SZ, [_I32, _I32, _I32]),
    "eval_ssim_sk": (C.c_int, [_P, _P, _P, _I32, _I32, _I32, _I32, _P, _SZ, _P, _P]),
    "lpips_packed_floats": (C.c_int64, [_I32, _I32]),
    "lpips_pack_weights": (C.c_int, [_P, _I32, _I32, _P, _P]),
    "lpips_tmp_bytes": (_SZ, [_I32, _I32]),
    "lpips_vgg": (C.c_int, [_P, _P, _P, _I32, _I32, _I32, _I32, _P, _P, _P, _P, _SZ, _P, _P]),
    "lpips_conv3x3_relu": (C.c_int, [_P, _P, _P, _I32, _I32, _I32, _I32, _I32, _P, _P]),
    "lpips_maxpool2": (C.c_int, [_P, _I64, _I32, _I32, _P, _P]),
    "lpips_distance_tmp_bytes": (_SZ, [_I32, _I32]),
    "lpips_distance": (C.c_int, [_P, _P, _P, _I32, _I32, _I32, _P, _SZ, _P, _P]),
    "depth_vis_tmp_bytes": (_SZ, [_I32, _I32]),
    "depth_vis": (C.c_int, [_P, _P, _I32, _I32, _I32, _P, _P, _SZ, _P, _P, _P, _P, _P]),
    "wef_tmp_bytes": (_SZ, [_I32, _I32, _I32, _I32]),
    "wef_maps": (C.c_int, [_P, _P, _I32, _I32, _I32, _I32, _P, _SZ, _P, _P, _P]),
    "wef_grid": (C.c_int, [_P, _I32, _I32, _I32, _P, _I32, _I32, _P, _P, _P]),
    "charbonnier_tmp_bytes": (_SZ, [_I64]),
    "charbonnier_fwd": (C.c_int, [_P, _P, _I64, C.c_double, _P, _SZ, _P, _P]),
    "charbonnier_bwd": (C.c_int, [_P, _P, _I64, C.c_double, _P, _P, _P, _P]),
    "depth_scales_tmp_bytes": (_SZ, [_I64]),
    "depth_scales": (C.c_int, [_P, _I64, _P, _P, _I64, _P, _P, _P, _P, _I32, _I32, _I32, _P, _SZ, _P, _P]),
    "invdepth_prepare": (C.c_int, [_P, _I32, _I32, _I32, _I32, _I32, C.c_float, _I32, C.c_float, C.c_float, C.c_float, _P, _P, _P]),
    "image_ingest_tmp_bytes": (_SZ, [_I32, _I32, _I32, _I32, _I32, _I32]),
    "image_ingest": (C.c_int, [_P, _I32, _I32, _I32, _I32, _I32, _P, _P, _I32, _P, _P, _I32, _I32, _P, _SZ, _P, _P, _P, _P]),
}

DEVICE_ONLY = ("export_row_mask", "backward_step", "backward_step_x", "backward_step_fsgs", "step_uninstanced", "export_tile_order", "export_tile_stop_depth", "forward_status", "forward_bin", "export_binning_region", "region_coop", "debug_blend_stats", "adam_step_gated", "tile_depth_limit_floats", "profile_enable", "profile_only", "profile_reset", "profile_stage_count", "profile_stage_name", "profile_read",
               "forward_render_x", "backward_x", "forward_tile_order",
               "image_stage_partials_count", "image_stage_fwd", "image_stage_bwd", "exposure_adam",
               "lgdwt_fused_fwd", "lgdwt_fused_bwd",
               "grid_encode_tmp_bytes", "grid_encode_fwd", "grid_encode_bwd", "sh_encode_fwd", "sh_encode_bwd",
               "depth_norm_tmp_bytes", "depth_norm_fwd", "depth_norm_bwd", "depth_smooth_fwd", "depth_smooth_bwd",
               "dng_depth_reg_fwd", "dng_depth_reg_bwd",
               "pearson_tmp_bytes", "pearson_fwd", "pearson_bwd",
               "dng_heads_tmp_bytes", "dng_heads_fwd", "dng_heads_bwd",
               "dng_reg_tmp_bytes", "dng_reg_fwd", "dng_reg_bwd", "view_dirs_fwd", "view_dirs_bwd", "near_mask",
               "dtu_mask", "masked_tmp_bytes", "masked_fill_fwd", "masked_fill_bwd", "alpha_penalty_fwd", "alpha_penalty_bwd",
               "dng_colour_rule",
               "blender_tmp_bytes", "blender_target", "dng_white_rule", "dng_white_rule_sh",
               "densify_tmp_bytes", "densify_plan", "densify_emit", "morton_codes", "densify_gather",
               "densify_fsgs_tmp_bytes", "densify_fsgs_plan", "densify_fsgs_merge", "densify_fsgs_emit", "densify_fsgs_prox_plan",
               "densify_fsgs_final", "densify_fsgs_gather",
               "densify_plan_gated", "prune_tmp_bytes", "prune_plan", "prune_emit",
               "eval_partials_count", "eval_tmp_bytes", "eval_metrics",
               "resize_tmp_bytes", "resize_bicubic_u8", "eval_ssim_sk_tmp_bytes", "eval_ssim_sk",
               "lpips_packed_floats", "lpips_pack_weights", "lpips_tmp_bytes", "lpips_vgg", "lpips_conv3x3_relu",
               "lpips_maxpool2", "lpips_distance_tmp_bytes", "lpips_distance",
               "depth_vis_tmp_bytes", "depth_vis",
               "wef_tmp_bytes", "wef_maps", "wef_grid", "charbonnier_tmp_bytes", "charbonnier_fwd", "charbonnier_bwd",
               "depth_scales_tmp_bytes", "depth_scales", "invdepth_prepare",
               "image_ingest_tmp_bytes", "image_ingest",
               "depth_forward", "depth_backward",
               "depth_backward_step",
               "adam_step_tensors", "backward_split",
               "debug_sort_tmp_bytes", "debug_sort_pairs", "debug_scan_sums")

ERRORS = {-1: "GS_E_NULL", -2: "GS_E_SHAPE", -3: "GS_E_SCRATCH", -4: "GS_E_OVERFLOW", -5: "GS_E_UNSUPPORTED"}


class GsError(RuntimeError):
    def __init__(self, fn, code):
        self.code = code
        what = ERRORS.get(code, "hipError_t %d" % code if code > 0 else "error %d" % code)
        super().__init__("%s failed: %s" % (fn, what))


class CApi:

    def __init__(self, path, prefix="gs_", optional=()):
        if not os.path.exists(path):
            raise ImportError(
                "gsplat native library not found at %s - build it first (python __graft_entry__.py "
                "or `make -C sparse-view-3dgs-pack_amd/csrc`); there is no fallback path." % path)
        self.path = path
        self.prefix = prefix
        self.lib = C.CDLL(path)
        self.missing = []
        for name, (res, args) in PROTOTYPES.items():
            try:
                f = getattr(self.lib, prefix + name)
            except AttributeError:
                if name in optional:
                    self.missing.append(name)
                    continue
                raise ImportError("%s does not export %s%s" % (path, prefix, name))
            f.restype = res
            f.argtypes = args
            setattr(self, "_" + name, f)

    def call(self, name, *args):
        rc = getattr(self, "_" + name)(*args)
        if rc != 0:
            raise GsError(self.prefix + name, rc)

    def raw(self, name):
        return getattr(self, "_" + name)


def read_profile(api):
    n = api.raw("profile_stage_count")()
    ms = (C.c_double * n)()
    cnt = (C.c_int64 * n)()
    api.call("profile_read", ms, cnt, n)
    return {api.raw("profile_stage_name")(i).decode(): (ms[i], cnt[i]) for i in range(n) if cnt[i] > 0}
```

sparse-view-3dgs-pack_amd/gsplat_amd/raster.py:

```python
import ctypes as C
import os

import torch

from .capi import GsGaussians, GsGrads, GsScratch, GsView

NUM_CHANNELS = 3
_DEPTH_ONLY = 2


def _ptr(t):
    if t is None or t.numel() == 0:
        return None
    return t.data_ptr()


def _prep(t, device):
    if t is None or t.numel() == 0:
        return None
    if t.dtype != torch.float32:
        t = t.float()
    if t.device != device:
        t = t.to(device)
    return t.contiguous()


def _regions(W, H):
    return ((((W + 15) // 16) + 3) // 4) * ((((H + 15) // 16) + 3) // 4)


class _Forward:
    __slots__ = ("device", "stream", "view", "g", "P", "W", "H", "geom", "img", "radii", "out_color", "out_invdepth",
                 "out_extra", "fsgs", "extra", "cache", "use_order", "use_limit", "static", "cur", "status")

    def __init__(self, device, stream, view, g, P, W, H, geom, img, radii, out_color, out_invdepth, out_extra, fsgs, extra,
                 cache, use_order, use_limit, static):
        self.device, self.stream, self.view, self.g = device, stream, view, g
        self.P, self.W, self.H = P, W, H
        self.geom, self.img, self.radii = geom, img, radii
        self.out_color, self.out_invdepth, self.out_extra = out_color, out_invdepth, out_extra
        self.fsgs, self.extra = fsgs, extra
        self.cache, self.use_order, self.use_limit, self.static = cache, use_order, use_limit, static
        self.cur = self.status = None


class _Last:
    __slots__ = ("geom", "P", "view", "g", "keep", "raw", "step", "radii", "img", "done")

    def __init__(self, geom, P, view, g, keep, raw):
        self.geom, self.P, self.view, self.g, self.keep, self.raw = geom, P, view, g, keep, raw
        self.step = self.radii = self.img = self.done = None


class RasterBackend:

    def __init__(self, api, device_type="cuda"):
        self.api = api
        self.device_type = device_type
        self._pinned = None
        self._capacity_hint = 0
        self._capacity_hint_limited = 0
        self.optimistic = os.environ.get("GS_SYNC_FORWARD", "0") != "1"
        self.tile_cull = os.environ.get("GS_TILE_CULL", "1") != "0"
        self.binning = os.environ.get("GS_BINNING", "auto")
        self.last_deferred_num_rendered = None
        self._region_off = set()
        self._cap_memo = {}
        self._scratch_memo = {}
        self._cap_by_buffer = {}
        self._cam_cache = {}
        self.camera_key = None
        self.camera_key_limits = False
        self._vm_ids = {}
        self.camera_cache_stats = dict(hits=0, misses=0, hashed=0)
        self.order_hint_on = True
        self.depth_limit_on = os.environ.get("GS_DEPTH_LIMIT", "0") == "1"
        self.depth_limit_request = None
        self.deferred = None
        self._status_ring = {}
        self.depth_limit_stats = dict(used=0, failed=0)
        self._pinned_by_device = {}
        self.grad_arena = None
        self.static_capacity = None
        self.static_step_tag = None
        self.fused_step = None
        self._side_streams = {}
        self._rows_ws = {}
        self.rows_epoch = 0
        self._last = None
        self.two_phase_launches = 0
        self._uninst_done = None
        self.raw_activations = False
        self.sh_rest = None
        self.sh_rest_activated = False
        self.keep_workspace = False
        self.last_workspace = None
        self._zero_images = {}

    def _stream(self, device):
        if device.type == "cuda":
            return C.c_void_p(torch.cuda.current_stream(device).cuda_stream)
        return None

    def _check_device(self, t):
        if t.device.type != self.device_type:
            raise RuntimeError(
                "gsplat %s backend got a tensor on %s - the rasterizer has no fallback path"
                % (self.device_type, t.device))

    def _tile_cull(self, device):
        cull = int(self.tile_cull)
        if cull and self.binning in ("region", "auto") and device.type == "cuda":
            return 2
        return cull

    def _view(self, keep, device, bg, viewmatrix, projmatrix, campos, tanfovx, tanfovy, H, W, scale_modifier,
              degree, prefiltered, antialiasing, debug, tile_cull=None):
        v = GsView()
        v.image_height, v.image_width = int(H), int(W)
        v.tanfovx, v.tanfovy = float(tanfovx), float(tanfovy)
        v.scale_modifier = float(scale_modifier)
        v.sh_degree = int(degree)
        v.prefiltered, v.antialiasing, v.debug = int(bool(prefiltered)), int(bool(antialiasing)), int(bool(debug))
        if self.force_rowwise_entries:
            v.debug |= 2
        v.tile_cull = self._tile_cull(device) if tile_cull is None else tile_cull
        bg, viewmatrix, projmatrix, campos = (_prep(x, device) for x in (bg, viewmatrix, projmatrix, campos))
        keep += [bg, viewmatrix, projmatrix, campos]
        v.bg, v.viewmatrix, v.projmatrix, v.campos = _ptr(bg), _ptr(viewmatrix), _ptr(projmatrix), _ptr(campos)
        return v

    def _gauss(self, keep, device, means3D, sh, colors, opacities, scales, rotations, cov3D, extra=None, raw=False,
               extra_gain=None, sh_rest=None):
        g = GsGaussians()
        g.raw_activations = int(bool(raw))
        extra = _prep(extra, device)
        keep.append(extra)
        g.extra_channel = _ptr(extra)
        if extra_gain is not None:
            extra_gain = _prep(extra_gain, device)
            keep.append(extra_gain)
            g.extra_gain = _ptr(extra_gain)
        means3D, sh, colors, opacities, scales, rotations, cov3D = (
            _prep(x, device) for x in (means3D, sh, colors, opacities, scales, rotations, cov3D))
        keep += [means3D, sh, colors, opacities, scales, rotations, cov3D]
        g.P = int(means3D.shape[0]) if means3D is not None else 0
        g.M = int(sh.shape[1]) if sh is not None else 0
        if sh_rest is not None:
            if sh is None or int(sh.shape[1]) != 1 or sh_rest.shape[0] != sh.shape[0]:
                raise RuntimeError("sh_rest goes with sh = the DC rows [P,1,3]")
            sh_rest = _prep(sh_rest, device)
            keep.append(sh_rest)
            g.M = 1 + int(sh_rest.shape[1])
            g.shs_rest = _ptr(sh_rest)
        g.means3D, g.shs, g.colors_precomp, g.opacities = _ptr(means3D), _ptr(sh), _ptr(colors), _ptr(opacities)
        g.scales, g.rotations, g.cov3D_precomp = _ptr(scales), _ptr(rotations), _ptr(cov3D)
        return g

    def _update_hint(self, num_rendered, limited=False):
        import math
        old = self._capacity_hint_limited if limited else self._capacity_hint
        want = max(int(num_rendered * 1.25) + 4096, int(old * 0.98))
        new = int(2.0 ** (math.ceil(math.log2(want) * 8.0) / 8.0))
        if limited:
            self._capacity_hint_limited = new
        else:
            self._capacity_hint = new

    def _remember_capacity(self, binning, cap):
        if len(self._cap_by_buffer) > 256:
            self._cap_by_buffer.clear()
        self._cap_by_buffer[(binning.data_ptr(), binning.numel())] = int(cap)

    def _capacity_of(self, P, W, H, nbytes, at_least):
        key = (P, W, H, nbytes)
        cap = self._cap_memo.get(key)
        if cap is None:
            lo, hi = int(at_least), max(int(at_least), 1)
            while self.scratch_bytes(P, W, H, hi)[2] <= nbytes:
                lo, hi = hi, hi * 2
            while lo < hi - 1:
                mid = (lo + hi) // 2
                if self.scratch_bytes(P, W, H, mid)[2] <= nbytes:
                    lo = mid
                else:
                    hi = mid
            cap = lo
            if len(self._cap_memo) > 64:
                self._cap_memo.clear()
            self._cap_memo[key] = cap
        return cap

    def last_num_rendered(self):
        return None if self._pinned is None else int(self._pinned[0])

    def take_deferred(self):
        d, self.deferred = self.deferred, None
        if d is None:
            return None

        def verdict():
            d["event"].synchronize()
            st = tuple(int(x) for x in d["status"][:4])
            ok = st[1] == 0 and st[2] == 0
            regions = d["regions"]
            if regions:
                if st[3] > self.REGION_MAX_ENTRIES:
                    self._region_off.add(d["size"])
                self._update_hint(max(st[0], st[3] * regions), limited=True)
                self.last_deferred_num_rendered = st[0]
            if not ok:
                self.depth_limit_stats["failed"] += 1
                if st[2] != 0 or not regions:
                    d["cache"]["limit_ok"] = False
                if st[2] != 0:
                    self.limits_failed(d["cache"])
            else:
                self.limits_held(d["cache"])
            return ok
        return verdict

    def last_status(self):
        return None if self._pinned is None else tuple(int(x) for x in self._pinned[:3])

    def _capacity_for(self, binning, P, W, H, R):
        if binning.numel() == 0:
            return R
        cap = self._cap_by_buffer.get((binning.data_ptr(), binning.numel()))
        if cap is not None and cap >= R:
            return cap
        return self._capacity_of(P, W, H, binning.numel(), R)

    def scratch_bytes(self, P, W, H, R):
        key = (int(P), int(W), int(H), int(R))
        memo = self._scratch_memo
        got = memo.get(key)
        if got is None:
            out = (C.c_size_t * 3)()
            ws = C.c_size_t(0)
            self.api.call("scratch_bytes", P, W, H, R, out, C.byref(ws))
            if len(memo) > 256:
                memo.clear()
            got = memo[key] = (out[0], out[1], out[2], ws.value)
        return got

    def _camera_identity(self, viewmatrix):
        ck, self.camera_key = self.camera_key, None
        if ck is not None:
            return ("key", ck)
        import hashlib
        import weakref
        ent = self._vm_ids.get(id(viewmatrix))
        if ent is not None and ent[0]() is viewmatrix and ent[1] == viewmatrix._version:
            return ent[2]
        self.camera_cache_stats["hashed"] += 1
        ident = ("hash", hashlib.blake2b(viewmatrix.detach().to("cpu", torch.float32).contiguous().numpy().tobytes(),
                                         digest_size=8).hexdigest())
        if len(self._vm_ids) > 1024:
            self._vm_ids = {k: v for k, v in self._vm_ids.items() if v[0]() is not None}
        try:
            self._vm_ids[id(viewmatrix)] = (weakref.ref(viewmatrix), viewmatrix._version, ident)
        except TypeError:
            pass
        return ident

    def _camera_cache(self, device, W, H, viewmatrix):
        if device.type != "cuda" or not (self.order_hint_on or self.depth_limit_on or self.depth_limit_request is not None
                                         or self.static_capacity is not None or self.camera_key_limits):
            self.camera_key = None
            return None
        key = (device.index, W, H, self._camera_identity(viewmatrix))
        c = self._cam_cache.get(key)
        if c is None:
            self.camera_cache_stats["misses"] += 1
            if len(self._cam_cache) >= self.CAMERA_CACHE_MAX:
                for k in self._cam_cache:
                    if not self._cam_cache[k].get("pinned"):
                        self._cam_cache.pop(k)
                        break
            T = ((W + 15) // 16) * ((H + 15) // 16)
            per_xcd = (T + 7) // 8
            b = torch.arange(per_xcd * 8, dtype=torch.int64)
            default_order = ((b & 7) * per_xcd + (b >> 3)).to(torch.int32)
            c = self._cam_cache[key] = dict(order=default_order.to(device), order_ok=False,
                                            limit=torch.full((int(self.api.raw("tile_depth_limit_floats")(W, H)),), float("inf"),
                                                             dtype=torch.float32, device=device),
                                            limit_ok=False, key=key,
                                            slack=torch.ones((1,), dtype=torch.float32, device=device), slack_level=0, held=0)
        else:
            self.camera_cache_stats["hits"] += 1
        return c

    CAMERA_CACHE_MAX = 256

    def drop_camera_entries(self, key_prefix):
        n = len(key_prefix)
        for k in [k for k in self._cam_cache if k[3][0] == "key" and isinstance(k[3][1], tuple) and k[3][1][:n] == key_prefix]:
            self._cam_cache.pop(k, None)

    def camera_entry(self, W, H, viewmatrix=None, camera_key=None, device_index=None):
        if camera_key is not None:
            ident = ("key", camera_key)
        else:
            saved, self.camera_key = self.camera_key, None
            hashed = self.camera_cache_stats["hashed"]
            ident = self._camera_identity(viewmatrix)
            self.camera_key, self.camera_cache_stats["hashed"] = saved, hashed
        if device_index is None:
            device_index = viewmatrix.device.index if viewmatrix is not None and viewmatrix.is_cuda else torch.cuda.current_device()
        return self._cam_cache.get((device_index, int(W), int(H), ident))

    SLACK = (1.0, 1.25, 1.6, 2.5)
    SLACK_RELAX_AFTER = 24

    def limits_failed(self, c):
        if c is None:
            return
        c["held"] = 0
        if c["slack_level"] < len(self.SLACK) - 1:
            c["slack_level"] += 1
            c["slack"].fill_(self.SLACK[c["slack_level"]])

    def limits_held(self, c):
        if c is None:
            return
        c["held"] += 1
        if c["held"] >= self.SLACK_RELAX_AFTER and c["slack_level"] > 0:
            c["held"] = 0
            c["slack_level"] -= 1
            c["slack"].fill_(self.SLACK[c["slack_level"]])

    @staticmethod
    def _scratch(geom, img=None, binning=None, capacity=0):
        s = GsScratch()
        s.geom, s.geom_bytes = _ptr(geom), geom.numel()
        if img is not None:
            s.img, s.img_bytes = _ptr(img), img.numel()
        if binning is not None:
            s.binning, s.binning_bytes = _ptr(binning), binning.numel()
        s.binning_capacity = int(capacity)
        return s

    force_rowwise_entries = False

    @property
    def region_coop(self):
        return bool(self.api.raw("region_coop")(-1))

    @region_coop.setter
    def region_coop(self, on):
        self.api.raw("region_coop")(int(bool(on)))

    scratch_fill = None
    output_fill = None
    KEYED_LIMITS = os.environ.get("GS_KEYED_LIMITS", "1") != "0"
    STATUS_IN_RENDER = True

    def _side_stream(self, device):
        side = self._side_streams.get(device.index)
        if side is None:
            side = self._side_streams[device.index] = torch.cuda.Stream(device=device)
        return side
    TWO_PHASE = os.environ.get("GS_TWO_PHASE_STEP", "1") != "0"
    TWO_PHASE_MIN_P = 100_000
    REACHED_SPLIT = os.environ.get("GS_REACHED_SPLIT", "1") != "0"

    def _two_phase(self, step, P):
        return self.TWO_PHASE and P >= self.TWO_PHASE_MIN_P and not step.grad_out[0]

    def _arms_side_launch(self, step, P):
        return self._two_phase(step, P) and not step.rows_override

    def launch_uninstanced_early(self):
        f = self._last
        if f is None or f.step is None or f.done is not None:
            return False
        f.done = self._launch_uninstanced(f.geom.device, f.view, f.g, f.radii, self._scratch(f.geom, f.img), f.step)
        return True

    def _structs(self, device, bg, means3D, sh, colors_precomp, opacities, scales, rotations, cov3D_precomp, viewmatrix,
                 projmatrix, campos, tanfovx, tanfovy, H, W, scale_modifier, degree, antialiasing, debug, extra=None, raw=False,
                 extra_gain=None, sh_rest=None):
        keep = []
        view = self._view(keep, device, bg, viewmatrix, projmatrix, campos, tanfovx, tanfovy, H, W, scale_modifier, degree,
                          False, antialiasing, debug)
        g = self._gauss(keep, device, means3D, sh, colors_precomp, opacities, scales, rotations, cov3D_precomp, extra, raw=raw,
                        extra_gain=extra_gain, sh_rest=sh_rest)
        return view, g, keep

    def _launch_uninstanced(self, device, view, g, radii, s, step):
        main = torch.cuda.current_stream(device)
        side = self._side_stream(device)
        side.wait_stream(main)
        step.reached_split = int(self.REACHED_SPLIT)
        self.api.call("step_uninstanced", C.byref(view), C.byref(g), radii.contiguous().data_ptr(), C.byref(s),
                      C.byref(step), C.c_void_p(side.cuda_stream))
        done = torch.cuda.Event()
        done.record(side)
        self.two_phase_launches += 1
        return done

    def rasterize_gaussians(self, bg, means3D, colors_precomp, opacities, scales, rotations, scale_modifier,
                            cov3D_precomp, viewmatrix, projmatrix, tanfovx, tanfovy, image_height, image_width,
                            sh, degree, campos, prefiltered, antialiasing, debug, extra=None, fsgs=False, extra_gain=None):
        if fsgs and (extra is not None or antialiasing):
            raise RuntimeError("the FSGS rasterizer generation has neither anti-aliasing nor a 4th channel")
        if means3D.ndim != 2 or means3D.shape[1] != 3:
            raise RuntimeError("means3D must have dimensions (num_points, 3)")
        self._check_device(means3D)
        device = means3D.device
        P, H, W = int(means3D.shape[0]), int(image_height), int(image_width)
        f32 = dict(dtype=torch.float32, device=device)
        u8 = dict(dtype=torch.uint8, device=device)
        alloc = torch.empty if P != 0 else torch.zeros
        out_color = alloc((NUM_CHANNELS, H, W), **f32)
        out_invdepth = alloc((1, H, W), **f32)
        radii = alloc((P,), dtype=torch.int32, device=device)
        out_extra = None if (extra is None and not fsgs) else alloc((1, H, W), **f32)
        tail = () if out_extra is None else (out_extra,)
        if self.output_fill is not None and P != 0:
            for kind, t in (("color", out_color), ("invdepth", out_invdepth), ("radii", radii), ("extra", out_extra)):
                if t is not None:
                    self.output_fill(kind, t)
        raw, self.raw_activations = self.raw_activations, False
        sh_rest, self.sh_rest = self.sh_rest, None
        sh_activated, self.sh_rest_activated = self.sh_rest_activated, False
        self._last = None
        if P == 0:
            self.camera_key, self.camera_key_limits, self.depth_limit_request = None, False, None
            e = torch.empty((0,), **u8)
            return (0, out_color, radii, e, e.clone(), e.clone(), out_invdepth) + tail
        if sh_rest is not None and not raw and (not sh_activated or fsgs or extra is not None):
            raise RuntimeError("split SH rows are served with raw activations only (gsplat_amd.render_raw), or on activated "
                               "values by the plain rasterizer call of gsplat_amd.accel")
        if fsgs and self.fused_step is not None:
            closed = None
            if self.static_capacity is not None:
                closed = "the capture-safe forward (GraphedStep, hipGraph replay) is"
            elif self.depth_limit_request is not None or self.depth_limit_on or self.camera_key_limits:
                closed = "depth-limited lists are"
            if closed is not None:
                self.fused_step, self.depth_limit_request, self.camera_key, self.camera_key_limits = None, None, None, False
                raise RuntimeError("%s closed to the fused train step of the FSGS rasterizer generation" % closed)
        if (extra_gain is not None) != (raw and extra is not None):
            raise RuntimeError("extra_gain goes with a RAW 4th channel (raw activations), and only with it")
        if device.type == "cuda":
            self._join_tile_order(device)
        cache = self._camera_cache(device, W, H, viewmatrix)
        static = self.static_capacity is not None
        request, self.depth_limit_request = self.depth_limit_request, None
        keyed_limits, self.camera_key_limits = self.camera_key_limits and self.KEYED_LIMITS, False
        self.deferred = None
        use_limit = cache is not None and (self.depth_limit_on or request is not None or keyed_limits) and self.tile_cull
        limit = cache["limit"] if use_limit and (static or cache["limit_ok"]) else None

        tile_cull = self._tile_cull(device)
        if tile_cull == 2 and ((P, W, H, limit is not None) in self._region_off or (
                self.binning == "auto" and limit is None and not static
                and self._capacity_hint > self.REGION_AUTO_MAX * _regions(W, H))):
            tile_cull = 1
        keep = []
        view = self._view(keep, device, bg, viewmatrix, projmatrix, campos, tanfovx, tanfovy, H, W, scale_modifier,
                          degree, prefiltered, antialiasing, debug, tile_cull=tile_cull)
        g = self._gauss(keep, device, means3D, sh, colors_precomp, opacities, scales, rotations, cov3D_precomp, extra, raw=raw,
                        extra_gain=extra_gain, sh_rest=sh_rest)

        gb, ib, _, _ = self.scratch_bytes(P, W, H, 0)
        geom = torch.empty((gb,), **u8)
        img = torch.empty((ib,), **u8)
        if self.scratch_fill is not None:
            self.scratch_fill("geom", geom)
            self.scratch_fill("img", img)
        last = self._last = _Last(geom, P, view, g, keep, raw)
        step = self.fused_step
        if step is not None and not fsgs and device.type == "cuda" and self._arms_side_launch(step, P):
            last.step, last.radii, last.img = step, radii, img
        f = _Forward(device, self._stream(device), view, g, P, W, H, geom, img, radii, out_color, out_invdepth, out_extra, fsgs,
                     extra, cache, cache is not None and self.order_hint_on, use_limit, static)

        if device.type != "cuda":
            nr = (C.c_int32 * 1)()
            self.api.call("forward_geometry", C.byref(view), C.byref(g), C.byref(self._scratch_of(f, None, 0, None)),
                          radii.data_ptr(), C.cast(nr, C.c_void_p), f.stream)
            num_rendered = int(nr[0])
            binning = self._new_binning(f, num_rendered)
            self._render(f, self._scratch_of(f, binning, num_rendered, None))
            return (num_rendered, out_color, radii, geom, binning, img, out_invdepth) + tail

        f.cur = torch.cuda.current_stream(device)
        pkey = (device.index, "static" if static else f.cur.cuda_stream)
        status = self._pinned_by_device.get(pkey)
        if status is None:
            status = self._pinned_by_device[pkey] = torch.zeros((16,), dtype=torch.int32).pin_memory()
        self._pinned = f.status = status
        num_rendered, binning = self._forward_lists(f, limit, request == "defer")
        return (num_rendered, out_color, radii, geom, binning, img, out_invdepth) + tail

    REGION_MAX_ENTRIES = 16384
    REGION_AUTO_MAX = 13000

    def _forward_lists(self, f, limit, defer):
        for lim in ((limit, None) if limit is not None else (None,)):
            deferred = defer and lim is not None and not f.static
            block = self._status_block(f.device) if deferred else (f.status if f.static else None)
            if f.view.tile_cull == 2:
                num_rendered, binning, s = self._lists_region(f, lim, block)
                if binning is None:
                    f.view.tile_cull = 1
                    return self._forward_lists(f, limit, defer)
            else:
                num_rendered, binning, s = self._lists_lsd(f, lim)
            if lim is not None:
                self.depth_limit_stats["used"] += 1
            if block is not None:
                if not s.status_host:
                    self.api.call("forward_status", C.byref(s), block.data_ptr(), f.stream)
                if deferred:
                    if s.defer_tile_order:
                        done = self._tile_order_on_side(f.view, s, f.cur)
                    else:
                        done = torch.cuda.Event()
                        done.record(f.cur)
                    self.deferred = dict(status=block, event=done, cache=f.cache, size=(f.P, f.W, f.H, True),
                                         regions=_regions(f.W, f.H) if f.view.tile_cull == 2 else 0)
            elif lim is not None:
                self.api.call("forward_status", C.byref(s), f.status.data_ptr(), f.stream)
                f.cur.synchronize()
                if int(f.status[2]) != 0:
                    self.depth_limit_stats["failed"] += 1
                    f.cache["limit_ok"] = False
                    self.limits_failed(f.cache)
                    del binning
                    continue
                self.limits_held(f.cache)
            if f.use_order:
                f.cache["order_ok"] = True
            if f.use_limit:
                f.cache["limit_ok"] = True
            return num_rendered, binning

    def _lists_lsd(self, f, limit):
        self.api.call("forward_geometry", C.byref(f.view), C.byref(f.g), C.byref(self._scratch_of(f, None, 0, limit)),
                      f.radii.data_ptr(), f.status.data_ptr(), f.stream)
        if f.static:
            cap = int(self.static_capacity)
            binning = self._new_binning(f, cap)
            s = self._scratch_of(f, binning, cap, limit)
            self._render(f, s)
            return cap, binning, s
        cap = self._capacity_hint if self.optimistic else 0
        if cap > 0 and limit is not None and self._capacity_hint_limited > 0:
            cap = self._capacity_hint_limited
        binning = None
        if cap > 0:
            ev = torch.cuda.Event()
            ev.record(f.cur)
            binning = self._new_binning(f, cap)
            s = self._scratch_of(f, binning, cap, limit)
            self._render(f, s)
            ev.synchronize()
        else:
            f.cur.synchronize()
        num_rendered = int(f.status[0])
        self._update_hint(num_rendered, limited=limit is not None)
        if binning is None or num_rendered > cap:
            binning = self._new_binning(f, num_rendered)
            s = self._scratch_of(f, binning, num_rendered, limit)
            self._render(f, s)
        return num_rendered, binning, s

    def _lists_region(self, f, limit, block):
        regions = _regions(f.W, f.H)
        limited = limit is not None
        if f.static:
            cap = int(self.static_capacity)
        else:
            hint = self._capacity_hint_limited if (limited and self._capacity_hint_limited > 0) else self._capacity_hint
            cap = hint if hint > 0 else max(8 * f.P, 1 << 20)
        for attempt in range(6):
            cap = max(cap, regions)
            binning = self._new_binning(f, cap)
            s = self._scratch_of(f, binning, cap, limit)
            self.api.call("forward_geometry", C.byref(f.view), C.byref(f.g), C.byref(s), f.radii.data_ptr(), None, f.stream)
            if block is not None:
                self.api.call("forward_bin", C.byref(f.view), C.byref(f.g), C.byref(s), None, f.stream)
                if self.STATUS_IN_RENDER:
                    s.status_host = block.data_ptr()
                    if self.fused_step is not None and not f.static:
                        s.defer_tile_order = 1
                self._render(f, s)
                return cap, binning, s
            self.api.call("forward_bin", C.byref(f.view), C.byref(f.g), C.byref(s), f.status.data_ptr(), f.stream)
            ev = torch.cuda.Event()
            ev.record(f.cur)
            self._render(f, s)
            ev.synchronize()
            st = tuple(int(x) for x in f.status[:4])
            if st[1] == 0:
                break
            if st[3] > self.REGION_MAX_ENTRIES:
                self._region_off.add((f.P, f.W, f.H, limited))
                return 0, None, None
            cap = int(max(st[0], st[3] * regions) * 1.25) + 4096
            del binning
        else:
            raise RuntimeError("region binning: the capacity did not settle (status %r)" % (st,))
        self._update_hint(max(st[0], st[3] * regions), limited=limited)
        return st[0], binning, s

    def _status_block(self, device):
        ring = self._status_ring.setdefault(device.index, [[], 0])
        if len(ring[0]) < 8:
            ring[0].append(torch.zeros((16,), dtype=torch.int32).pin_memory())
        block = ring[0][ring[1] % len(ring[0])]
        ring[1] += 1
        return block

    def _new_binning(self, f, cap):
        _, _, bb, _ = self.scratch_bytes(f.P, f.W, f.H, cap)
        binning = torch.empty((bb,), dtype=torch.uint8, device=f.device)
        if self.scratch_fill is not None:
            self.scratch_fill("binning", binning)
        self._remember_capacity(binning, cap)
        return binning

    def _scratch_of(self, f, binning, capacity, limit):
        s = self._scratch(f.geom, f.img, binning, capacity)
        if limit is not None:
            s.tile_depth_limit = limit.data_ptr()
        if f.static and self.static_step_tag is not None:
            s.step_tag = self.static_step_tag.data_ptr()
        return s

    def _render(self, f, scratch):
        c = f.cache
        if f.use_order:
            if c["order_ok"]:
                scratch.tile_order_hint = c["order"].data_ptr()
            scratch.tile_order_out = c["order"].data_ptr()
        if f.use_limit:
            scratch.tile_depth_limit_out = c["limit"].data_ptr()
            scratch.tile_depth_limit_slack = c["slack"].data_ptr()
        if f.fsgs == _DEPTH_ONLY:
            self.api.call("depth_forward", C.byref(f.view), C.byref(f.g), C.byref(scratch), f.out_invdepth.data_ptr(),
                          f.out_extra.data_ptr(), f.stream)
        elif f.fsgs:
            self.api.call("forward_render_fsgs", C.byref(f.view), C.byref(f.g), C.byref(scratch), f.out_color.data_ptr(),
                          f.out_invdepth.data_ptr(), f.out_extra.data_ptr(), f.stream)
        elif f.extra is None:
            self.api.call("forward_render", C.byref(f.view), C.byref(f.g), C.byref(scratch), f.out_color.data_ptr(),
                          f.out_invdepth.data_ptr(), f.stream)
        else:
            self.api.call("forward_render_x", C.byref(f.view), C.byref(f.g), C.byref(scratch), f.out_color.data_ptr(),
                          f.out_invdepth.data_ptr(), f.out_extra.data_ptr(), f.stream)

    def _tile_order_on_side(self, view, scratch, main):
        side = self._side_stream(main.device)
        ev = torch.cuda.Event()
        ev.record(main)
        side.wait_event(ev)
        self.api.call("forward_tile_order", C.byref(view), C.byref(scratch), C.c_void_p(side.cuda_stream))
        done = torch.cuda.Event()
        done.record(side)
        self._tile_order_done = done
        return done
# ... 13 lines not shown
        f32 = dict(dtype=torch.float32, device=device)
        alloc = torch.empty if P != 0 else torch.zeros
        depth, alpha = alloc((1, H, W), **f32), alloc((1, H, W), **f32)
        radii = alloc((P,), dtype=torch.int32, device=device)
        if P == 0:
            return depth, alpha, radii, None
        tile_cull = self._tile_cull(device)
        if tile_cull == 2 and ((P, W, H, False) in self._region_off or (
                self.binning == "auto" and self._capacity_hint > self.REGION_AUTO_MAX * _regions(W, H))):
            tile_cull = 1
        keep = []
        view = self._view(keep, device, bg, viewmatrix, projmatrix, campos, tanfovx, tanfovy, H, W, scale_modifier, 0, False,
                          False, debug, tile_cull=tile_cull)
        g = self._gauss(keep, device, means3D, None, means3D, opacities, scales, rotations, cov3D_precomp)
        gb, ib, _, _ = self.scratch_bytes(P, W, H, 0)
        u8 = dict(dtype=torch.uint8, device=device)
        geom, img = torch.empty((gb,), **u8), torch.empty((ib,), **u8)
        if self.scratch_fill is not None:
            self.scratch_fill("geom", geom)
            self.scratch_fill("img", img)
        f = _Forward(device, self._stream(device), view, g, P, W, H, geom, img, radii, None, depth, alpha, _DEPTH_ONLY, None,
                     None, False, False, False)
        f.cur = torch.cuda.current_stream(device)
        pkey = (device.index, f.cur.cuda_stream)
        status = self._pinned_by_device.get(pkey)
        if status is None:
            status = self._pinned_by_device[pkey] = torch.zeros((16,), dtype=torch.int32).pin_memory()
        f.status = status
        num_rendered, binning = self._forward_lists(f, None, False)
        return depth, alpha, radii, dict(view=f.view, g=g, keep=keep, radii=radii, geom=geom, img=img, binning=binning,
                                         R=int(num_rendered), P=P, W=W, H=H)

    def depth_backward(self, rec, dL_ddepth, dL_dalpha, grad_flags, workspace=None):
        device = rec["radii"].device
        P, W, H, R = rec["P"], rec["W"], rec["H"], rec["R"]
        f32 = dict(dtype=torch.float32, device=device)
        dL_ddepth, dL_dalpha = _prep(dL_ddepth, device), _prep(dL_dalpha, device)
        dm3 = torch.empty((P, 3), **f32) if grad_flags & 1 else None
        dm2 = torch.empty((P, 3), **f32) if grad_flags & 1 else None
        dop = torch.empty((P, 1), **f32) if grad_flags & 2 else None
        ws = workspace
        if ws is None:
            ws = torch.empty((((P * 128 + 255) // 256) * 256,), dtype=torch.uint8, device=device)
        binning = rec["binning"]
        s = self._scratch(rec["geom"], rec["img"], binning, self._capacity_for(binning, P, W, H, R))
        self.api.call("depth_backward", C.byref(rec["view"]), C.byref(rec["g"]), rec["radii"].data_ptr(), C.byref(s), R,
                      _ptr(dL_ddepth), _ptr(dL_dalpha), int(grad_flags), _ptr(dm3), _ptr(dm2), _ptr(dop), ws.data_ptr(),
                      ws.numel(), self._stream(device))
        return dm3, dm2, dop

    def depth_backward_step(self, rec, dL_ddepth, dL_dalpha, which, param, exp_avg, exp_avg_sq, lr, step, betas=(0.9, 0.999),
                            eps=1e-15, flags=0, workspace=None):
        device = rec["radii"].device
        P, W, H, R = rec["P"], rec["W"], rec["H"], rec["R"]
        if not hasattr(self.api, "_depth_backward_step"):
            raise RuntimeError("the loaded library has no gs_depth_backward_step - there is no fallback")
        for name, t in (("param", param), ("exp_avg", exp_avg), ("exp_avg_sq", exp_avg_sq)):
            if t.device != device or t.dtype != torch.float32 or not t.is_contiguous() or t.numel() != P * (3 if which == 1 else 1):
                raise RuntimeError("depth_backward_step: %s must be a contiguous fp32 tensor of %d rows on %s" % (name, P, device))
        dL_ddepth, dL_dalpha = _prep(dL_ddepth, device), _prep(dL_dalpha, device)
        ws = workspace
        if ws is None:
            ws = torch.empty((((P * 128 + 255) // 256) * 256,), dtype=torch.uint8, device=device)
        binning = rec["binning"]
        s = self._scratch(rec["geom"], rec["img"], binning, self._capacity_for(binning, P, W, H, R))
        self.api.call("depth_backward_step", C.byref(rec["view"]), C.byref(rec["g"]), rec["radii"].data_ptr(), C.byref(s), R,
                      _ptr(dL_ddepth), _ptr(dL_dalpha), int(which), param.data_ptr(), exp_avg.data_ptr(), exp_avg_sq.data_ptr(),
                      float(lr), int(step), float(betas[0]), float(betas[1]), float(eps), int(flags), ws.data_ptr(), ws.numel(),
                      self._stream(device))

    def rasterize_gaussians_backward(self, bg, means3D, radii, colors_precomp, opacities, scales, rotations,
                                     scale_modifier, cov3D_precomp, viewmatrix, projmatrix, tanfovx, tanfovy,
                                     dL_dout_color, dL_dout_invdepth, sh, degree, campos, geomBuffer, R,
                                     binningBuffer, imgBuffer, antialiasing, debug, extra=None, dL_dout_extra=None,
                                     fsgs=False, extra_gain=None, raw=False):
        self._check_device(means3D)
        device = means3D.device
        P = int(means3D.shape[0])
        H, W = int(dL_dout_color.shape[1]), int(dL_dout_color.shape[2])
        if device.type == "cuda":
            self._join_tile_order(device)
        arena, self.grad_arena = self.grad_arena, None
        step, self.fused_step = self.fused_step, None
        sh_rest, self.sh_rest = self.sh_rest, None
        sh_activated, self.sh_rest_activated = self.sh_rest_activated, False
        f = self._last if self._last is not None and self._last.geom is geomBuffer else None
        if f is not None:
            raw = f.raw
        split = sh_rest is not None and sh_activated and step is None and not raw and not fsgs and extra is None
        if sh_rest is not None and not split and (step is None or not raw or not step.grad_out_rest):
            raise RuntimeError("split SH rows: the backward is gs_backward_split (activated values, no 4th channel) or "
                               "gs_backward_step's gradients-out form with grad_out_rest")
        if raw and (step is None or P == 0):
            raise RuntimeError("a forward on raw activations must be followed by the fused train-step backward")
        fused = step is not None and P != 0
        if fused and fsgs and not hasattr(self.api, "_backward_step_fsgs"):
            raise RuntimeError("this library has no fused train-step backward for the FSGS rasterizer generation")
        dL_dout_color, dL_dout_invdepth = _prep(dL_dout_color, device), _prep(dL_dout_invdepth, device)
        if extra is not None:
            dL_dout_extra = _prep(dL_dout_extra, device)
            if dL_dout_extra is None:
                dL_dout_extra = torch.zeros((1, H, W), dtype=torch.float32, device=device)
        elif not fsgs:
            dL_dout_extra = None
        if fused and f is not None:
            view, g = f.view, f.g
        else:
            view, g, keep = self._structs(device, bg, means3D, sh, colors_precomp, opacities, scales, rotations, cov3D_precomp,
                                          viewmatrix, projmatrix, campos, tanfovx, tanfovy, H, W, scale_modifier, degree,
                                          antialiasing, debug, extra, raw=raw, extra_gain=extra_gain if raw else None,
                                          sh_rest=sh_rest)
        args = (view, g, radii.contiguous(), geomBuffer, binningBuffer, imgBuffer, P, W, H, R, dL_dout_color, dL_dout_invdepth,
                dL_dout_extra)
        if fused:
            return self._backward_step(step, f, *args, fsgs=fsgs)
        return self._backward_grads(arena, fsgs, *args)

    def _zero_image(self, device, H, W):
        key = (device.index, H, W)
        z = self._zero_images.get(key)
        if z is None:
            if len(self._zero_images) > 8:
                self._zero_images.clear()
            z = self._zero_images[key] = torch.zeros((1, H, W), dtype=torch.float32, device=device)
        return z

    def _backward_step_fsgs(self, step, view, g, radii, geom, binning, img, P, W, H, R, dL_dout_color, dL_ddepth, dL_dalpha):
        device = radii.device
        if step.phase != 0 or step.phase1_done:
            raise RuntimeError("the two-phase step (side launch of gs_step_uninstanced) is closed to the FSGS rasterizer "
                               "generation")
        if step.extra:
            raise RuntimeError("the FSGS rasterizer generation has no 4th channel to step")
        _, _, _, wsb = self.scratch_bytes(P, W, H, R)
        ws = self._rows_workspace(step, device, wsb)
        s = self._scratch(geom, img, binning, self._capacity_for(binning, P, W, H, R))
        last = self._last
        if last is not None:
            last.step = last.radii = last.img = last.done = None
        step.reached_split = int(self.REACHED_SPLIT)
        dL_ddepth, dL_dalpha = _prep(dL_ddepth, device), _prep(dL_dalpha, device)
        zeros = self._zero_image(device, H, W) if dL_ddepth is None or dL_dalpha is None else None
        try:
            self.api.call("backward_step_fsgs", C.byref(view), C.byref(g), radii.data_ptr(), C.byref(s), int(R),
                          dL_dout_color.data_ptr(), (dL_ddepth if dL_ddepth is not None else zeros).data_ptr(),
                          (dL_dalpha if dL_dalpha is not None else zeros).data_ptr(), C.byref(step), _ptr(ws), ws.numel(),
                          self._stream(device))
        except Exception:
            self.rows_epoch += 1
            raise
        if step.rows_clean:
            self._rows_ws[(device.index, wsb)][1] = True
        return (None,) * 8

    def _backward_step(self, step, f, view, g, radii, geom, binning, img, P, W, H, R, dL_dout_color, dL_dout_invdepth,
                       dL_dout_extra, fsgs=False):
        if fsgs:
            return self._backward_step_fsgs(step, view, g, radii, geom, binning, img, P, W, H, R, dL_dout_color,
                                            dL_dout_invdepth, dL_dout_extra)
        device = radii.device
        _, _, _, wsb = self.scratch_bytes(P, W, H, R)
        ws = self._rows_workspace(step, device, wsb)
        s = self._scratch(geom, img, binning, self._capacity_for(binning, P, W, H, R))
        done, last = None, self._last
        if last is not None:
            if last is f and last.step is step:
# ... 191 lines not shown
```

sparse-view-3dgs-pack_amd/gsplat_amd/trainer.py:

```python
import math

import torch
import torch.distributed as dist

FIELDS = (("xyz", 3), ("features", 48), ("opacity", 1), ("scaling", 3), ("rotation", 4))
FLOATS_PER_GAUSSIAN = sum(n for _, n in FIELDS)
LRS = {"xyz": 0.00016, "f_dc": 0.0025, "f_rest": 0.0025 / 20.0, "opacity": 0.025, "scaling": 0.005, "rotation": 0.001,
       "nir_albedo": 0.00016, "nir_gain": 0.0025}
NIR_FIELD = ("nir_albedo", 1)
SHARD_UNIT = 4 * 840


def expon_lr(step, lr_init, lr_final, lr_delay_steps=0, lr_delay_mult=1.0, max_steps=1000000):
    import numpy as np
    if step < 0 or (lr_init == 0.0 and lr_final == 0.0):
        return 0.0
    if lr_delay_steps > 0:
        delay_rate = lr_delay_mult + (1 - lr_delay_mult) * np.sin(0.5 * np.pi * np.clip(step / lr_delay_steps, 0, 1))
    else:
        delay_rate = 1.0
    t = np.clip(step / max_steps, 0, 1)
    log_lerp = np.exp(np.log(lr_init) * (1 - t) + np.log(lr_final) * t)
    return float(delay_rate * log_lerp)

# ... 1035 lines not shown


class TrainOptions:

    def __init__(self, **kw):
        self.iterations = 30_000
        self.position_lr_final = 0.0000016
        self.position_lr_delay_mult = 0.01
        self.position_lr_max_steps = 30_000
        self.densification_interval = 100
        self.opacity_reset_interval = 3000
        self.densify_from_iter = 500
        self.densify_until_iter = 15_000
        self.densify_grad_threshold = 0.0002
        self.min_opacity = 0.005
        self.size_threshold = 20
        self.sh_increase_interval = 1000
        self.depth_l1_weight_init = 1.0
        self.depth_l1_weight_final = 0.01
        self.optimizer_type = "default"
        self.white_background = False
        self.random_background = False
        self.cameras_extent = 1.0
        self.seed = 0
        self.densify_on_device = False
        self.densify_rule = "3dgs"
        self.dist_thres = 10.0
        self.prune_from_iter = 500
        self.proximity_until_iter = 2000
        self.split_opacity_thresh = 0.1
        for k, v in kw.items():
            if not hasattr(self, k):
                raise TypeError("unknown option %s" % k)
            setattr(self, k, v)


def cameras_extent(camera_centers):
    c = torch.stack([torch.as_tensor(x, dtype=torch.float64).reshape(3) for x in camera_centers])
    return float((c - c.mean(dim=0, keepdim=True)).norm(dim=1).max() * 1.1)


class Trainer:

    def __init__(self, model, cameras, gt_images, criterion, Rasterizer, Settings, bg, rank=0, world_size=1,
                 optimizer_step=True, masks=None, sharded_optimizer=None, sparse_exchange=None, optimizer_type="default",
                 alpha_masks=None):
        import os
        self.sharded_optimizer = (os.environ.get("GS_SHARDED_ADAM", "1") == "1") if sharded_optimizer is None \
            else bool(sharded_optimizer)
        self.sparse_exchange = (os.environ.get("GS_SPARSE_EXCHANGE", "0") == "1") if sparse_exchange is None \
            else bool(sparse_exchange)
        self.last_exchange = None
        if optimizer_type not in ("default", "sparse_adam"):
            raise ValueError("optimizer_type must be 'default' or 'sparse_adam'")
        self.optimizer_type = optimizer_type
        if optimizer_type == "sparse_adam":
            if not isinstance(model.optimizer, FlatAdam):
                raise RuntimeError("sparse_adam needs the flat Adam state (a model built with an api)")
            model.optimizer.sparse = True
            self.sharded_optimizer = False
        self.model, self.cameras, self.gts, self.criterion = model, cameras, gt_images, criterion
        self.Rasterizer, self.Settings, self.bg = Rasterizer, Settings, bg
        self.rank, self.world_size = rank, world_size
        self.optimizer_step = optimizer_step
        self.masks = masks
        self.alpha_masks = alpha_masks
        self._bg_gen = None
        self.depth_priors = None
        self.depth_l1_weight = 0.0
        self.last = None
        Trainer._uids = getattr(Trainer, "_uids", 0) + 1
        self.uid = Trainer._uids
        be = getattr(getattr(getattr(self.Rasterizer, "_fn", None), "_impl", None), "backend", None)
        if be is not None and hasattr(be, "drop_camera_entries"):
            import weakref
            weakref.finalize(self, be.drop_camera_entries, ("trainer", self.uid))
        self._stack = []
        self._rng = None

    def camera_index(self, k):
        return (k * self.world_size + self.rank) % len(self.cameras)

    def step(self, k):
        return self._step_camera(self.camera_index(k), self.optimizer_step, ())

    def draw_cameras(self, seed):
        import random
        if self._rng is None:
            self._rng = random.Random(seed)
        mine = None
        for r in range(self.world_size):
            if not self._stack:
                self._stack = list(range(len(self.cameras)))
            ci = self._stack.pop(self._rng.randint(0, len(self._stack) - 1))
            if r == self.rank:
                mine = ci
        return mine

    densify_decisions = None
    last_options = None
    alpha_masks = None
    _bg_gen = None
    _use_stage = False

    def train_iteration(self, iteration, opt):
        self.sync()
        self.last_options = opt
        m = self.model
        m.update_learning_rate(iteration, opt.position_lr_final, opt.position_lr_delay_mult, opt.position_lr_max_steps,
                               exposure_max_steps=opt.iterations)
        if iteration % opt.sh_increase_interval == 0:
            m.oneupSHdegree()
        if self.depth_priors is not None:
            self.depth_l1_weight = expon_lr(iteration, opt.depth_l1_weight_init, opt.depth_l1_weight_final, max_steps=opt.iterations)
        ci = self.draw_cameras(opt.seed)
        if opt.random_background:
            self._draw_background(opt.seed)
        in_densify = iteration < opt.densify_until_iter
        will_densify = in_densify and iteration > opt.densify_from_iter and iteration % opt.densification_interval == 0
        will_reset = in_densify and (iteration % opt.opacity_reset_interval == 0 or
                                     (opt.white_background and iteration == opt.densify_from_iter))
        do_step = iteration < opt.iterations and not will_densify
        loss = self._step_camera(ci, do_step, ("opacity",) if will_reset else (), exposure_step=iteration < opt.iterations)
        if will_densify or will_reset or iteration >= opt.iterations:
            self.sync()
        densified, reset = None, False
        if will_densify:
            self.gather_optimizer_state()
            thr = opt.size_threshold if iteration > opt.opacity_reset_interval else None
            dec = self.densify_decisions(iteration) if self.densify_decisions is not None else None
            densified = self._densify(iteration, opt, opt.min_opacity, thr, radii=self.last["radii"], decisions=dec)
        if will_reset:
            m.reset_opacity()
            reset = True
        return dict(loss=loss, densified=densified, reset=reset, P=m.P, camera=ci)

    def _densify(self, iteration, opt, min_opacity, max_screen_size, rule=None, radii=None, decisions=None):
        m = self.model
        gen = torch.Generator().manual_seed(opt.seed * 1000003 + iteration)
        on_device = bool(getattr(opt, "densify_on_device", False))
        rule = rule or getattr(opt, "densify_rule", "3dgs")
        if rule == "fsgs":
            return m.densify_and_prune_fsgs(opt.densify_grad_threshold, min_opacity, opt.cameras_extent, None, iteration,
                                            dist_thres=opt.dist_thres, prune_from_iter=opt.prune_from_iter,
                                            proximity_until_iter=opt.proximity_until_iter, generator=gen, on_device=on_device)
        if rule == "3dgs":
            return m.densify_and_prune(opt.densify_grad_threshold, min_opacity, opt.cameras_extent, max_screen_size, radii,
                                       generator=gen, decisions=decisions, on_device=on_device)
        if rule == "dng":
            return m.densify_and_prune_dng(opt.densify_grad_threshold, min_opacity, opt.cameras_extent, None,
                                           opt.split_opacity_thresh, None, generator=gen, on_device=on_device)
        raise ValueError("densify_rule must be '3dgs', 'fsgs' or 'dng'")

    def _draw_background(self, seed):
        if self._bg_gen is None:
            dev = self.bg.device if torch.is_tensor(self.bg) else torch.device(self.model.device)
            self._bg_gen = torch.Generator(device=dev)
            self._bg_gen.manual_seed(int(seed) + self.rank)
            self.bg = torch.empty((3,), dtype=torch.float32, device=dev)
        torch.rand((3,), out=self.bg, generator=self._bg_gen)

    def _alpha(self, ci):
        return None if self.alpha_masks is None else self.alpha_masks[ci]

    def _image_extras(self):
        return self.model.exposure is not None or self.alpha_masks is not None or self._bg_gen is not None

    def _stage_ok(self):
        from .optim import ExposureAdam
        m = self.model
        return (self.optimizer_type != "sparse_adam" and type(self)._render_view is Trainer._render_view
                and type(self)._criterion_backward is Trainer._criterion_backward
                and (m.exposure is None or isinstance(m.exposure_optimizer, ExposureAdam)))

    FUSED_STEP = __import__("os").environ.get("GS_FUSED_STEP", "1") != "0"

    def _fused_step_ok(self, backend, optimizer_step):
        m = self.model
        return (self.FUSED_STEP and optimizer_step and self.world_size == 1 and backend is not None
                and isinstance(m.optimizer, FlatAdam) and (not m.with_nir or self.RENDERS_NIR) and m.flat.is_cuda
                and hasattr(backend.api, "_backward_step") and hasattr(backend, "fused_step"))

    RENDERS_NIR = False

    def _fused_dp_ok(self, backend, optimizer_step):
        m = self.model
        return (self.FUSED_STEP and optimizer_step and self.world_size > 1 and backend is not None
                and isinstance(m.optimizer, FlatAdam) and (not m.with_nir or self.RENDERS_NIR) and m.flat.is_cuda
                and hasattr(backend.api, "_backward_step") and hasattr(backend.api, "_adam_step_gated")
                and hasattr(backend, "fused_step"))

    depth_limit = None
    RAW_ACTIVATIONS = True

    def sync(self):
        g = getattr(self, "_graphed", None)
        if g is not None:
            g.settle()
        p, self._pending = getattr(self, "_pending", None), None
        if p is None:
            return
        if "flag_host" in p:
            p["event"].synchronize()
            if p["verdict"] is not None:
                p["verdict"]()
            if float(p["flag_host"][0]) == 0.0:
                return
        elif p["verdict"]():
            return
        opt = self.model.optimizer
        opt.t, opt.seg_steps = p["counters"][0], dict(p["counters"][1])
        if p.get("exposure_steps") is not None:
            self.model.exposure_optimizer.steps = p["exposure_steps"]
        if p["running_mean"] is not None:
            self.criterion.dwt_running_mean.copy_(p["running_mean"])
        p["loss"].copy_(self._step_camera(p["ci"], True, p["skip"], exposure_step=p.get("exposure_step")))
        self.sync()

    def checkpoint(self):
        self.sync()
        self.gather_optimizer_state()
        return self.model.capture()

    def _backend(self):
        be = getattr(getattr(self.Rasterizer, "_fn", None), "_impl", None)
        return getattr(be, "backend", None)

    _EVAL_KEEPS = ("_capacity_hint", "_capacity_hint_limited", "_last", "last_workspace", "_pinned", "deferred",
                   "last_deferred_num_rendered")

    def evaluate(self, cameras=None, gts=None, **kw):
        from .evaluate import evaluate_views
        self.sync()
        cameras = self.cameras if cameras is None else cameras
        gts = self.gts if gts is None else gts
        be = self._backend()
        saved = {k: getattr(be, k) for k in self._EVAL_KEEPS if be is not None and hasattr(be, k)}
        try:
            return evaluate_views(self.model, cameras, gts, self.Rasterizer, self.Settings, self.bg,
                                  camera_keys=[("trainer", self.uid, "eval", i) for i in range(len(cameras))], **kw)
        finally:
            for k, v in saved.items():
                setattr(be, k, v)

    def wef_report(self, camera=0, bands="level2", path=None, titled=False, tile_cols=3):
        from . import wef
        if bands not in ("level2", "all"):
            raise ValueError("wef_report: bands is 'level2' or 'all' (got %r)" % (bands,))
        if type(self).evaluate is not Trainer.evaluate:
            raise NotImplementedError("wef_report renders as Trainer.evaluate does; %s renders its views differently" % type(self).__name__)
        self.sync()
        ci = int(camera)
        be = self._backend()
        saved = {k: getattr(be, k) for k in self._EVAL_KEEPS if be is not None and hasattr(be, k)}
        try:
            with torch.no_grad():
                img = render(self.cameras[ci], self.model, self.Rasterizer, self.Settings, self.bg, filter_as_indices=None,
                             clamp=False, camera_key=("trainer", self.uid, "eval", ci))["render"].clamp(0, 1)
        finally:
            for k, v in saved.items():
                setattr(be, k, v)
        gt = self.gts[ci].to(img.device)
        maps = wef.compute_wef_all_subbands(img, gt) if bands == "all" else wef.compute_wef_maps(img, gt)
        grid = (wef.make_wef_grid_image_titled if titled else wef.make_wef_grid_image)(maps, list(maps), tile_cols=tile_cols)
        if path is not None:
            from .imageio import write_png
            write_png(path, grid)
        return dict(maps, grid=grid)

    def _before_relayout(self, on_device, opt):
        self.sync()
        self.gather_optimizer_state()
        if on_device is None:
            on_device = getattr(opt if opt is not None else self.last_options, "densify_on_device", False)
        return bool(on_device)

    def prune_near_cameras(self, centers, near_range, on_device=None, opt=None):
        on_device = self._before_relayout(on_device, opt)
        m = self.model
        with torch.no_grad():
            xyz = m.params["xyz"].detach()
            centers = torch.as_tensor(centers, dtype=torch.float32).reshape(-1, 3).to(xyz.device)
            if xyz.is_cuda:
                from .dng_reg import near_camera_mask
                mask = near_camera_mask(xyz, centers, near_range)
            else:
                mask = None
                for c in centers:
                    near = (xyz - c.repeat(xyz.shape[0], 1)).norm(dim=1, keepdim=True) < near_range
                    mask = mask + near if mask is not None else near
                mask = mask.squeeze(1)
        return m.prune_points(mask, on_device=on_device)

    def prune_unseen(self, camera_indices=None, on_device=None, opt=None):
        on_device = self._before_relayout(on_device, opt)
        m = self.model
        idx = range(len(self.cameras)) if camera_indices is None else list(camera_indices)
        be = self._backend()
        saved = {k: getattr(be, k) for k in self._EVAL_KEEPS if be is not None and hasattr(be, k)}
        seen = torch.zeros((m.P,), dtype=torch.bool, device=m.flat.device)
        try:
            with torch.no_grad():
                for ci in idx:
                    radii = render(self.cameras[ci], m, self.Rasterizer, self.Settings, self.bg, filter_as_indices=None,
                                   clamp=False, camera_key=("trainer", self.uid, "eval", ci))["radii"]
                    seen |= radii.reshape(-1) > 0
        finally:
            for k, v in saved.items():
                setattr(be, k, v)
        return m.prune_points(~seen, on_device=on_device)

    MANUAL_BACKWARD = __import__("os").environ.get("GS_MANUAL_BACKWARD", "1") != "0"

    class _ManualCtx:

        def __init__(self):
            self.saved_tensors = ()

        def save_for_backward(self, *tensors):
            self.saved_tensors = tensors

        def mark_non_differentiable(self, *a):
            pass

        def set_materialize_grads(self, v):
            pass

    def _manual_step_ok(self, fused_step, fused):
        fn = getattr(self.Rasterizer, "_fn", None)
        return (self.MANUAL_BACKWARD and fused_step and fused and (not self._image_extras() or self._stage_ok()) and fn is not None
                and getattr(getattr(fn, "_impl", None), "backend", None) is not None
                and type(self)._render_view is Trainer._render_view and type(self)._criterion_backward is Trainer._criterion_backward)

    def _manual_step(self, ci, mask, backend, deferred):
        m, cam = self.model, self.cameras[ci]
        fn = self.Rasterizer._fn
        rs = self.Settings(
            image_height=int(cam.image_height), image_width=int(cam.image_width), tanfovx=math.tan(cam.FoVx * 0.5),
            tanfovy=math.tan(cam.FoVy * 0.5), bg=self.bg, scale_modifier=1.0, viewmatrix=cam.world_view_transform,
            projmatrix=cam.full_proj_transform, sh_degree=m.active_sh_degree, campos=cam.camera_center, prefiltered=False,
            debug=False, antialiasing=False)
        backend.camera_key = ("trainer", self.uid, ci)
        backend.camera_key_limits = False
        empty = getattr(self, "_empty_cpu", None)
        if empty is None:
            empty = self._empty_cpu = torch.Tensor([])
        rctx, lctx = self._ManualCtx(), self._ManualCtx()
        with torch.no_grad():
            p = m.params
            color, radii, depth = fn.forward(rctx, p["xyz"], None, p["features"], empty, p["opacity"], p["scaling"], p["rotation"],
                                             empty, rs)
            verdict = backend.take_deferred() if deferred else None
            loss, parts = self.criterion.fused_call(color, self.gts[ci], mask=mask, manual_ctx=lctx,
                                                    exposure=None if m.exposure is None else m.exposure[ci], alpha=self._alpha(ci))
            grad_depth = None
            prior = self._depth_prior(ci)
            if prior is not None:
                dl, grad_depth = self.criterion.ops.depth_l1_step(depth, prior[0], prior[1], self.depth_l1_weight)
                loss = loss + dl
                parts = dict(parts, depth_l1=dl)
            self._arm_side_launch(backend.launch_uninstanced_early)
            from .losses import FusedLGDWTLoss
            grad_img = FusedLGDWTLoss.backward(lctx, self.criterion.ops.unit_grad(loss.device), None)[1]
            fn.backward(rctx, grad_img, None, grad_depth)
        pkg = {"render": color, "viewspace_points": None, "visibility_filter": None, "radii": radii, "depth": depth}
        return pkg, loss, parts, verdict

    def _render_view(self, ci, fused, raw):
        m = self.model
        return render(self.cameras[ci], m, self.Rasterizer, self.Settings, self.bg, filter_as_indices=None,
                      clamp=not fused, fused=True, use_trained_exp=m.exposure is not None and not self._use_stage, camera_index=ci,
                      raw_activations=raw, camera_key=("trainer", self.uid, ci))

    def load_depth_priors(self, keys, depths_dir, depth_params=None, resolutions=None, nerf_synthetic=False):
        from .depth_priors import load_depth_priors
        if resolutions is None:
            resolutions = [(int(g.shape[-1]), int(g.shape[-2])) for g in self.gts]
        self.depth_priors = load_depth_priors(keys, depths_dir, depth_params, resolutions, nerf_synthetic=nerf_synthetic,
                                              device=self.gts[0].device)
        return self.depth_priors

    def _depth_prior(self, ci):
        if self.depth_priors is None or not self.depth_l1_weight > 0:
            return None
        return self.depth_priors[ci]

    def _depth_term(self, pkg, ci, loss, parts):
        prior = self._depth_prior(ci)
        if prior is None:
            return loss, parts
        dl = self.depth_l1_weight * self.criterion.ops.depth_l1(pkg["depth"], prior[0], prior[1])
        return loss + dl, dict(parts, depth_l1=dl.detach())

    def _criterion_backward(self, pkg, ci, mask, fused, side_launch):
        alpha = self._alpha(ci)
        if self._use_stage:
            m = self.model
            loss, parts = self.criterion.fused_call(pkg["render"], self.gts[ci], mask=mask,
                                                    exposure=None if m.exposure is None else m.exposure.detach()[ci], alpha=alpha)
            loss, parts = self._depth_term(pkg, ci, loss, parts)
            self._arm_side_launch(side_launch)
            torch.autograd.backward(loss, self.criterion.ops.unit_grad(loss.device))
            return loss, parts
        if alpha is not None:
            pkg = dict(pkg, render=(pkg["render"].clamp(0, 1) if fused else pkg["render"]) * alpha.reshape(pkg["render"].shape[-2:]))
        if fused:
            loss, parts = self.criterion.fused_call(pkg["render"], self.gts[ci], mask=mask)
            loss, parts = self._depth_term(pkg, ci, loss, parts)
            self._arm_side_launch(side_launch)
            torch.autograd.backward(loss, self.criterion.ops.unit_grad(loss.device))
        else:
            loss, parts = self.criterion(pkg["render"], self.gts[ci], mask=mask)
            loss, parts = self._depth_term(pkg, ci, loss, parts)
            loss.backward()
        return loss, parts

    def _arm_side_launch(self, side_launch):
        self.criterion.ops.before_last_backward_kernel = side_launch

    def _unfused_tail(self, pkg, radii, optimizer_step, skip):
        m = self.model
        self.last_radii = radii
        with torch.no_grad():
            m.collect_grads()
            m.update_view_statistics(radii, pkg["viewspace_points"].grad, into_delta=self.world_size > 1)
            if self.world_size > 1:
                torch.gt(radii, 0, out=m.grad_mask.view(torch.bool))
            self.exchange_and_step(optimizer_step, skip)

    def _step_camera(self, ci, optimizer_step, skip, exposure_step=None):
        self.sync()
        m = self.model
        if exposure_step is None:
            exposure_step = optimizer_step
        m.zero_grad()
        backend = self._backend()
        fused_step = self._fused_step_ok(backend, optimizer_step)
        fused_dp = self._fused_dp_ok(backend, optimizer_step)
        fused = getattr(self.criterion, "fused", False)
        stage_ok = self._stage_ok()
        self._use_stage = bool(fused and (fused_step or fused_dp) and stage_ok
                               and (m.exposure is not None or self.alpha_masks is not None))
        deferred = (fused_step or fused_dp) and self.depth_limit == "deferred" and getattr(self, "_coef_dev", None) is None \
            and (not self._image_extras() or stage_ok)
        if deferred:
            counters = (m.optimizer.t, dict(m.optimizer.seg_steps))
            backend.depth_limit_request = "defer"
        if fused_dp:
            backend.raw_activations = self.RAW_ACTIVATIONS
            backend.fused_step = m.optimizer.grads_out_request()
            if not self.RAW_ACTIVATIONS:
                raise RuntimeError("the data-parallel fused backward takes the raw parameter rows (Trainer.RAW_ACTIVATIONS)")
        elif fused_step:
            backend.raw_activations = self.RAW_ACTIVATIONS
            backend.fused_step = m.optimizer.fused_request(skip, coef_dev=getattr(self, "_coef_dev", None))
            rows = getattr(self, "rows_override", None)
            if rows is not None:
                backend.fused_step.rows_override = rows.data_ptr()
            if self._use_stage and m.exposure is not None:
                backend.fused_step.fail_flag = m.exposure_optimizer.gate.data_ptr()
        elif backend is not None and hasattr(backend, "grad_arena") and not m.with_nir:
            m.arm_grad_arena(backend)
        mask = None if self.masks is None else self.masks[ci]
        rm = None
        path = "fused" if (fused_step or fused_dp) else "unfused"
        exp_steps = m.exposure_optimizer.steps if (self._use_stage and m.exposure is not None) else None
        if self.RAW_ACTIVATIONS and self._manual_step_ok(fused_step, fused):
            path = "manual"
            pkg, loss, parts, verdict = self._manual_step(ci, mask, backend, deferred)
        else:
            pkg = self._render_view(ci, fused, (fused_step or fused_dp) and self.RAW_ACTIVATIONS)
            verdict = backend.take_deferred() if deferred else None
            if self.world_size > 1 and self.sparse_exchange:
                if fused_dp and hasattr(backend, "export_row_mask") and backend.export_row_mask(m.union_mask):
                    self._begin_union()
                else:
                    self._begin_union(pkg["radii"] > 0)
            if verdict is not None and not fused:
                rm = getattr(self.criterion, "dwt_running_mean", None)
                rm = None if rm is None else rm.clone()
            loss, parts = self._criterion_backward(pkg, ci, mask, fused,
                                                   backend.launch_uninstanced_early if (fused_step and fused) else None)
        radii = pkg["radii"]
        if fused_dp:
            if backend.fused_step is not None:
                backend.fused_step = None
                raise RuntimeError("fused data-parallel step armed but the rasterizer backward did not run")
            with torch.no_grad():
                self.exchange_and_step(optimizer_step, skip, gate=m.fail_flag)
            if deferred:
                host = self._flag_blocks[self._flag_i % len(self._flag_blocks)] if getattr(self, "_flag_blocks", None) else None
                if host is None:
                    self._flag_blocks = [torch.zeros((1,), dtype=torch.float32).pin_memory() for _ in range(4)]
                    self._flag_i = 0
                    host = self._flag_blocks[0]
                self._flag_i += 1
                host.copy_(m.fail_flag, non_blocking=True)
                ev = torch.cuda.Event()
                ev.record(torch.cuda.current_stream(m.flat.device))
                if fused:
                    rm = parts.get("running_mean_before")
                self._pending = dict(verdict=verdict, flag_host=host, event=ev, ci=ci, skip=skip, counters=counters,
                                     running_mean=rm, loss=loss.detach(), exposure_steps=exp_steps, exposure_step=exposure_step)
        elif verdict is not None:
            if fused:
                rm = parts.get("running_mean_before")
            self._pending = dict(verdict=verdict, ci=ci, skip=skip, counters=counters, running_mean=rm, loss=loss.detach(),
                                 exposure_steps=exp_steps, exposure_step=exposure_step)
        if fused_dp:
            pass
        elif fused_step:
            if backend.fused_step is not None:
                backend.fused_step = None
                raise RuntimeError("fused train step armed but the rasterizer backward did not run")
        else:
            self._unfused_tail(pkg, radii, optimizer_step, skip)
        partials = parts.get("exposure_partials") if self._use_stage else None
        if partials is not None:
            eo = m.exposure_optimizer
            gate = m.fail_flag if fused_dp else eo.gate
            if self.world_size > 1:
                eo.grad_row(partials, ci)
                dist.all_reduce(m.exposure.grad, op=dist.ReduceOp.SUM)
                if exposure_step:
                    eo.step(gate=gate)
            elif exposure_step:
                eo.step_from_partials(partials, ci, gate=gate)
            else:
                eo.grad_row(partials, ci)
            eo.zero_grad(set_to_none=True)
        elif m.exposure_optimizer is not None:
            if m.exposure.grad is not None:
                if self.world_size > 1:
                    dist.all_reduce(m.exposure.grad, op=dist.ReduceOp.SUM)
                if exposure_step:
                    m.exposure_optimizer.step()
            m.exposure_optimizer.zero_grad(set_to_none=True)
        self.last = dict(loss=loss.detach(), radii=radii, parts=parts, path=path)
        return loss.detach()

    DP_CHUNKS = 4

    def exchange_and_step(self, optimizer_step, skip=(), gate=None):
# ... 1618 lines not shown
```

Measured before the change: 1280.

## Precompute next view's preprocess for unreached blocks on side stream during backward

Adds an early-geometry path that runs preprocess for the next camera, restricted to blocks whose Gaussians are not touched by the fused optimizer step, on a side stream while the current step finishes. The following forward then waits on an event and only reprocesses the blocks containing reached Gaussians, plus a reduced header reset. The goal is to overlap most of the preprocess with the backward/step tail and shorten the critical path. It adds token-based validity checks, event synchronization and fallback/drop logic, with a risk of stale data or contention on the side stream.

```diff
diff --git a/include/gsplat.h b/include/gsplat.h
--- a/include/gsplat.h
+++ b/include/gsplat.h
@@ -71,6 +71,7 @@
   const uint32_t* step_tag;
   const float* tile_depth_limit_slack;
   uint32_t* status_host;
+  void* early_geometry_done;
 } GsScratch;
 
 typedef struct GsGrads {
@@ -206,6 +207,9 @@
 
 int gs_step_uninstanced(const GsView* view, const GsGaussians* g, const int32_t* radii,
                         const GsScratch* scratch, const GsStepState* st, void* stream);
+
+int gs_forward_geometry_early(const GsView* view, const GsGaussians* g, const GsScratch* scratch, int32_t* radii,
+                              void* stream);
 
 int gs_backward_from_rows(const GsView* view, const GsGaussians* g, const int32_t* radii,
                           const GsScratch* scratch, const double* rows, int32_t depth_mode,
diff --git a/profiles/step_timeline.py b/profiles/step_timeline.py
--- /dev/null
+++ b/profiles/step_timeline.py
@@ -0,0 +1,43 @@
+#!/usr/bin/env python3
+import csv
+import glob
+import os
+import sys
+
+src, out = sys.argv[1], sys.argv[2]
+trace = glob.glob(os.path.join(src, "**", "*_kernel_trace.csv"), recursive=True)[0]
+tr = sorted(csv.DictReader(open(trace)), key=lambda r: int(r["Start_Timestamp"]))
+
+
+def short(name):
+    name = name.split("(")[0]
+    for cut in ("void ", "(anonymous namespace)::"):
+        name = name.replace(cut, "")
+    return name.split("<")[0][-48:]
+
+
+idx = [i for i, r in enumerate(tr) if "render_bwd_wave_kernel" in r["Kernel_Name"]]
+two = [j for j in range(1, len(idx)) if any("step_uninstanced_kernel" in r["Kernel_Name"] for r in tr[idx[j - 1]:idx[j]])]
+j = two[(2 * len(two)) // 3]
+a, b = idx[j - 1], idx[j]
+t0, t_end = int(tr[a]["Start_Timestamp"]), int(tr[b]["Start_Timestamp"])
+seg = [r for r in tr if int(r["End_Timestamp"]) > t0 and int(r["Start_Timestamp"]) < t_end and r is not tr[b]]
+iv = sorted((max(int(r["Start_Timestamp"]), t0), min(int(r["End_Timestamp"]), t_end)) for r in seg)
+busy, cs, ce = 0, None, None
+for s0, e0 in iv:
+    if ce is None or s0 > ce:
+        busy += (ce - cs) if ce is not None else 0
+        cs, ce = s0, e0
+    else:
+        ce = max(ce, e0)
+busy += (ce - cs) if ce is not None else 0
+queues = {}
+with open(out, "w") as f:
+    f.write("one steady-state train step (render_bwd to render_bwd), rocprofv3 --kernel-trace; start and duration in us\n")
+    f.write("wall %.3f ms, GPU busy %.3f ms, %d kernel launches\n" % ((t_end - t0) / 1e6, busy / 1e6, len(seg)))
+    f.write("%9s %9s %5s  %s\n" % ("start", "duration", "queue", "kernel"))
+    for r in seg:
+        q = queues.setdefault(r.get("Queue_Id", "?"), len(queues))
+        s0, e0 = int(r["Start_Timestamp"]), int(r["End_Timestamp"])
+        f.write("%9.1f %9.1f %5d  %s\n" % ((s0 - t0) / 1e3, (e0 - s0) / 1e3, q, short(r["Kernel_Name"])))
+print(open(out).read())
diff --git a/sparse-view-3dgs-pack_amd/csrc/gs_api.hip b/sparse-view-3dgs-pack_amd/csrc/gs_api.hip
--- a/sparse-view-3dgs-pack_amd/csrc/gs_api.hip
+++ b/sparse-view-3dgs-pack_amd/csrc/gs_api.hip
@@ -97,23 +97,9 @@
   return GS_OK;
 }
 
-int gs_forward_geometry(const GsView* v, const GsGaussians* g, GsScratch* sc, int32_t* radii,
-                        int32_t* num_rendered_host, void* stream) {
-  int rc = check_args(v, g);
-  if (rc) return rc;
-  if (!sc || !sc->geom) return GS_E_NULL;
-  sc->binned = 0;
-  hipStream_t s = (hipStream_t)stream;
+static int geometry_args(const GsView* v, const GsGaussians* g, const GsScratch* sc, int32_t* radii, PreprocessArgs& a,
+                         RegionLayout& rl) {
   const int P = g->P;
-  if (sc->geom_bytes < geom_bytes((size_t)P)) return GS_E_SCRATCH;
-  GeomView gv = geom_view(sc->geom, (size_t)P);
-  if (P == 0) {
-    GS_HIP_CHECK(hipMemsetAsync(gv.hdr, 0, sizeof(GeomHeader), s));
-    if (num_rendered_host) GS_HIP_CHECK(hipMemcpyAsync(num_rendered_host, &gv.hdr->num_rendered, 4, hipMemcpyDeviceToHost, s));
-    return GS_OK;
-  }
-  if (!radii) return GS_E_NULL;
-  PreprocessArgs a;
   a.P = P;
   a.D = v->sh_degree;
   a.M = g->M;
@@ -148,20 +134,52 @@
   a.region_cap = 0;
   a.rg_x = a.rg_y = 0;
   if (v->tile_cull == 2) {
-    RegionLayout rl;
-    rc = region_layout(v, sc, rl);
+    const int rc = region_layout(v, sc, rl);
     if (rc) return rc;
     a.region_count = rl.count;
     a.region_bucket = rl.bucket;
     a.region_cap = rl.cap;
     a.rg_x = rl.rg_x;
     a.rg_y = rl.rg_y;
+  }
+  return GS_OK;
+}
+
+int gs_forward_geometry(const GsView* v, const GsGaussians* g, GsScratch* sc, int32_t* radii,
+                        int32_t* num_rendered_host, void* stream) {
+  int rc = check_args(v, g);
+  if (rc) return rc;
+  if (!sc || !sc->geom) return GS_E_NULL;
+  sc->binned = 0;
+  void* const early_done = sc->early_geometry_done;
+  sc->early_geometry_done = nullptr;
+  hipStream_t s = (hipStream_t)stream;
+  const int P = g->P;
+  if (sc->geom_bytes < geom_bytes((size_t)P)) return GS_E_SCRATCH;
+  GeomView gv = geom_view(sc->geom, (size_t)P);
+  if (P == 0) {
+    GS_HIP_CHECK(hipMemsetAsync(gv.hdr, 0, sizeof(GeomHeader), s));
+    if (num_rendered_host) GS_HIP_CHECK(hipMemcpyAsync(num_rendered_host, &gv.hdr->num_rendered, 4, hipMemcpyDeviceToHost, s));
+    return GS_OK;
+  }
+  if (!radii) return GS_E_NULL;
+  if (early_done && (v->tile_cull != 2 || !reached_marking())) return GS_E_UNSUPPORTED;
+  PreprocessArgs a;
+  RegionLayout rl = {};
+  rc = geometry_args(v, g, sc, radii, a, rl);
+  if (rc) return rc;
+  if (early_done) {
+    const hipError_t e = hipStreamWaitEvent(s, (hipEvent_t)early_done, 0);
+    if (e != hipSuccess) return (int)e;
+    launch_region_prepare(gv, rl.count, rl.rg_x * rl.rg_y, (uint32_t)P, s, 2);
+    GS_LAUNCH_CHECK(s, v->debug);
+  } else if (v->tile_cull == 2) {
     launch_region_prepare(gv, rl.count, rl.rg_x * rl.rg_y, (uint32_t)P, s);
     GS_LAUNCH_CHECK(s, v->debug);
   }
   {
     GS_PROF(ST_PREPROCESS_FWD, s);
-    launch_preprocess_fwd(a, gv, s);
+    launch_preprocess_fwd(a, gv, s, early_done ? 2 : 0);
   }
   GS_LAUNCH_CHECK(s, v->debug);
   if (v->tile_cull != 2) {
@@ -171,6 +189,26 @@
   GS_LAUNCH_CHECK(s, v->debug);
   if (num_rendered_host)
     GS_HIP_CHECK(hipMemcpyAsync(num_rendered_host, &gv.hdr->num_rendered, 4, hipMemcpyDeviceToHost, s));
+  return GS_OK;
+}
+
+int gs_forward_geometry_early(const GsView* v, const GsGaussians* g, const GsScratch* sc, int32_t* radii, void* stream) {
+  int rc = check_args(v, g);
+  if (rc) return rc;
+  if (!sc || !sc->geom || !radii) return GS_E_NULL;
+  if (v->tile_cull != 2 || !reached_marking() || g->P == 0) return GS_E_UNSUPPORTED;
+  hipStream_t s = (hipStream_t)stream;
+  const int P = g->P;
+  if (sc->geom_bytes < geom_bytes((size_t)P)) return GS_E_SCRATCH;
+  GeomView gv = geom_view(sc->geom, (size_t)P);
+  PreprocessArgs a;
+  RegionLayout rl = {};
+  rc = geometry_args(v, g, sc, radii, a, rl);
+  if (rc) return rc;
+  launch_region_prepare(gv, rl.count, rl.rg_x * rl.rg_y, (uint32_t)P, s, 1);
+  GS_LAUNCH_CHECK(s, v->debug);
+  launch_preprocess_fwd(a, gv, s, 1);
+  GS_LAUNCH_CHECK(s, v->debug);
   return GS_OK;
 }
 
diff --git a/sparse-view-3dgs-pack_amd/csrc/gs_common.h b/sparse-view-3dgs-pack_amd/csrc/gs_common.h
--- a/sparse-view-3dgs-pack_amd/csrc/gs_common.h
+++ b/sparse-view-3dgs-pack_amd/csrc/gs_common.h
@@ -244,7 +244,7 @@
   uint32_t region_cap;
   int rg_x, rg_y;
 };
-int launch_preprocess_fwd(const PreprocessArgs& a, const GeomView& g, hipStream_t s);
+int launch_preprocess_fwd(const PreprocessArgs& a, const GeomView& g, hipStream_t s, int block_filter = 0);
 int launch_scan_block_sums(const GeomView& g, int P, hipStream_t s);
 int launch_mark_visible(int P, const float* means3D, const float* viewmatrix, uint8_t* present, hipStream_t s);
 
@@ -261,7 +261,7 @@
   const int64_t c = regions > 0 ? capacity / regions : 0;
   return (uint32_t)(c > RG_MAX_ENTRIES ? RG_MAX_ENTRIES : (c < 0 ? 0 : c));
 }
-int launch_region_prepare(const GeomView& g, uint32_t* region_count, int regions, uint32_t P, hipStream_t s);
+int launch_region_prepare(const GeomView& g, uint32_t* region_count, int regions, uint32_t P, hipStream_t s, int parts = 3);
 int launch_region_bin(const GeomView& g, const uint32_t* region_count, const uint2* region_bucket, uint32_t region_cap, int rg_x,
                       int rg_y, int grid_x, int grid_y, const float* tile_depth_limit, uint2* ranges, uint32_t* point_list,
                       int64_t capacity, hipStream_t s);
diff --git a/sparse-view-3dgs-pack_amd/csrc/gs_preprocess.hip b/sparse-view-3dgs-pack_amd/csrc/gs_preprocess.hip
--- a/sparse-view-3dgs-pack_amd/csrc/gs_preprocess.hip
+++ b/sparse-view-3dgs-pack_amd/csrc/gs_preprocess.hip
@@ -70,9 +70,20 @@
   uint32_t tiles[64];
 };
 
-template <bool COOP>
+#define PF_ALL 0
+#define PF_UNREACHED 1
+#define PF_REACHED 2
+template <bool COOP, int FILTER = PF_ALL>
 __global__ void __launch_bounds__(GS_BLOCK) preprocess_fwd_kernel(PreprocessArgs a, GeomView g, int lds_floats) {
   const int idx = blockIdx.x * GS_BLOCK + threadIdx.x;
+  if constexpr (FILTER != PF_ALL) {
+    const int has_reached = __syncthreads_or((idx < a.P && g.reached[idx] != 0) ? 1 : 0);
+    if (FILTER == PF_REACHED && idx == 0) {
+      g.hdr->pad[HDR_LIMITED] = a.tile_depth_limit ? 1u : 0u;
+      g.hdr->pad[HDR_REACHED] = 0u;
+    }
+    if ((has_reached != 0) != (FILTER == PF_REACHED)) return;
+  }
   uint32_t tiles = 0, entries = TB_ENTRIES_UNKNOWN;
   const int T = a.grid_x * a.grid_y;
   int p0 = 0, p1 = 0, p2 = 0, p3 = 0, n_pend = 0;
@@ -117,7 +128,7 @@
   asm volatile("" : "+v"(op_in), "+v"(sc_in.x), "+v"(sc_in.y), "+v"(sc_in.z), "+v"(rq_in.x), "+v"(rq_in.y), "+v"(rq_in.z),
                "+v"(rq_in.w));
   const GsLdsFloatPtr lds_seg = (GsLdsFloatPtr)s_limit + (GS_LIMIT_TILES_IN_LDS ? T : 0);
-  if (idx == 0) {
+  if (FILTER == PF_ALL && idx == 0) {
     g.hdr->pad[HDR_LIMITED] = a.tile_depth_limit ? 1u : 0u;
     g.hdr->pad[HDR_REACHED] = 0u;
   }
@@ -540,15 +551,21 @@
   return region_coop_form();
 }
 
-int launch_preprocess_fwd(const PreprocessArgs& a, const GeomView& g, hipStream_t s) {
+template <int FILTER>
+static void launch_preprocess_fwd_form(const PreprocessArgs& a, const GeomView& g, hipStream_t s) {
   const int nb = (a.P + GS_BLOCK - 1) / GS_BLOCK;
   const size_t lds = preprocess_limit_lds_floats(a);
   const bool coop = a.tile_cull == 2 && region_coop_form() && a.rg_x <= 0xFFFF && a.rg_y <= 0xFFFF &&
                     (long long)a.rg_x * a.rg_y <= (1ll << 26);
   if (coop)
-    hipLaunchKernelGGL(preprocess_fwd_kernel<true>, dim3(nb), dim3(GS_BLOCK), 4 * lds, s, a, g, (int)lds);
+    hipLaunchKernelGGL((preprocess_fwd_kernel<true, FILTER>), dim3(nb), dim3(GS_BLOCK), 4 * lds, s, a, g, (int)lds);
   else
-    hipLaunchKernelGGL(preprocess_fwd_kernel<false>, dim3(nb), dim3(GS_BLOCK), 4 * lds, s, a, g, (int)lds);
+    hipLaunchKernelGGL((preprocess_fwd_kernel<false, FILTER>), dim3(nb), dim3(GS_BLOCK), 4 * lds, s, a, g, (int)lds);
+}
+int launch_preprocess_fwd(const PreprocessArgs& a, const GeomView& g, hipStream_t s, int block_filter) {
+  if (block_filter == PF_UNREACHED) launch_preprocess_fwd_form<PF_UNREACHED>(a, g, s);
+  else if (block_filter == PF_REACHED) launch_preprocess_fwd_form<PF_REACHED>(a, g, s);
+  else launch_preprocess_fwd_form<PF_ALL>(a, g, s);
   return 0;
 }
 int launch_scan_block_sums(const GeomView& g, int P, hipStream_t s) {
diff --git a/sparse-view-3dgs-pack_amd/csrc/gs_regionbin.hip b/sparse-view-3dgs-pack_amd/csrc/gs_regionbin.hip
--- a/sparse-view-3dgs-pack_amd/csrc/gs_regionbin.hip
+++ b/sparse-view-3dgs-pack_amd/csrc/gs_regionbin.hip
@@ -5,11 +5,12 @@
 #define RB_WAVES (RB_THREADS / 64)
 #define RB_TILES (RG_TILES * RG_TILES)
 
+template <int PARTS>
 __global__ void __launch_bounds__(GS_BLOCK) region_prepare_kernel(GeomHeader* hdr, uint32_t* __restrict__ region_count,
                                                                    int regions, uint32_t P) {
   const int i = blockIdx.x * GS_BLOCK + threadIdx.x;
-  if (i < regions) region_count[(size_t)i * RG_COUNT_STRIDE] = 0u;
-  if (i == 0) {
+  if ((PARTS & 1) && i < regions) region_count[(size_t)i * RG_COUNT_STRIDE] = 0u;
+  if ((PARTS & 2) && i == 0) {
     hdr->num_rendered = 0u;
     hdr->overflow = 0u;
     hdr->trunc_failed = 0u;
@@ -189,9 +190,14 @@
     keys_sorted[i] = ((uint64_t)blockIdx.x << 32) | (uint64_t)__float_as_uint(splat[point_list[i]].depth);
 }
 
-int launch_region_prepare(const GeomView& g, uint32_t* region_count, int regions, uint32_t P, hipStream_t s) {
-  hipLaunchKernelGGL(region_prepare_kernel, dim3((regions + GS_BLOCK - 1) / GS_BLOCK > 0 ? (regions + GS_BLOCK - 1) / GS_BLOCK : 1),
-                     dim3(GS_BLOCK), 0, s, g.hdr, region_count, regions, P);
+int launch_region_prepare(const GeomView& g, uint32_t* region_count, int regions, uint32_t P, hipStream_t s, int parts) {
+  const dim3 grid((regions + GS_BLOCK - 1) / GS_BLOCK > 0 ? (regions + GS_BLOCK - 1) / GS_BLOCK : 1);
+  if (parts == 1)
+    hipLaunchKernelGGL(region_prepare_kernel<1>, grid, dim3(GS_BLOCK), 0, s, g.hdr, region_count, regions, P);
+  else if (parts == 2)
+    hipLaunchKernelGGL(region_prepare_kernel<2>, dim3(1), dim3(64), 0, s, g.hdr, region_count, regions, P);
+  else
+    hipLaunchKernelGGL(region_prepare_kernel<3>, grid, dim3(GS_BLOCK), 0, s, g.hdr, region_count, regions, P);
   return 0;
 }
 
diff --git a/sparse-view-3dgs-pack_amd/gsplat_amd/capi.py b/sparse-view-3dgs-pack_amd/gsplat_amd/capi.py
--- a/sparse-view-3dgs-pack_amd/gsplat_amd/capi.py
+++ b/sparse-view-3dgs-pack_amd/gsplat_amd/capi.py
@@ -59,6 +59,7 @@
         ("step_tag", C.c_void_p),
         ("tile_depth_limit_slack", C.c_void_p),
         ("status_host", C.c_void_p),
+        ("early_geometry_done", C.c_void_p),
     ]
 
 
@@ -144,6 +145,7 @@
                                       _P, _P, _P, _F, _I32, _F, _F, _F, _I32, _P, _SZ, _P]),
     "step_uninstanced": (C.c_int, [C.POINTER(GsView), C.POINTER(GsGaussians), _P, C.POINTER(GsScratch),
                                    C.POINTER(GsStepState), _P]),
+    "forward_geometry_early": (C.c_int, [C.POINTER(GsView), C.POINTER(GsGaussians), C.POINTER(GsScratch), _P, _P]),
     "backward_step": (C.c_int, [C.POINTER(GsView), C.POINTER(GsGaussians), _P, C.POINTER(GsScratch), _I64, _P, _P,
                                 C.POINTER(GsStepState), _P, _SZ, _P]),
     "backward_step_x": (C.c_int, [C.POINTER(GsView), C.POINTER(GsGaussians), _P, C.POINTER(GsScratch), _I64, _P, _P, _P,
@@ -307,7 +309,7 @@
     "image_ingest": (C.c_int, [_P, _I32, _I32, _I32, _I32, _I32, _P, _P, _I32, _P, _P, _I32, _I32, _P, _SZ, _P, _P, _P, _P]),
 }
 
-DEVICE_ONLY = ("export_row_mask", "backward_step", "backward_step_x", "backward_step_fsgs", "step_uninstanced", "export_tile_order", "export_tile_stop_depth", "forward_status", "forward_bin", "export_binning_region", "region_coop", "debug_blend_stats", "adam_step_gated", "tile_depth_limit_floats", "profile_enable", "profile_only", "profile_reset", "profile_stage_count", "profile_stage_name", "profile_read",
+DEVICE_ONLY = ("export_row_mask", "backward_step", "backward_step_x", "backward_step_fsgs", "step_uninstanced", "forward_geometry_early", "export_tile_order", "export_tile_stop_depth", "forward_status", "forward_bin", "export_binning_region", "region_coop", "debug_blend_stats", "adam_step_gated", "tile_depth_limit_floats", "profile_enable", "profile_only", "profile_reset", "profile_stage_count", "profile_stage_name", "profile_read",
                "forward_render_x", "backward_x", "forward_tile_order",
                "image_stage_partials_count", "image_stage_fwd", "image_stage_bwd", "exposure_adam",
                "lgdwt_fused_fwd", "lgdwt_fused_bwd",
diff --git a/sparse-view-3dgs-pack_amd/gsplat_amd/raster.py b/sparse-view-3dgs-pack_amd/gsplat_amd/raster.py
--- a/sparse-view-3dgs-pack_amd/gsplat_amd/raster.py
+++ b/sparse-view-3dgs-pack_amd/gsplat_amd/raster.py
@@ -31,7 +31,7 @@
 
 class _Forward:
     __slots__ = ("device", "stream", "view", "g", "P", "W", "H", "geom", "img", "radii", "out_color", "out_invdepth",
-                 "out_extra", "fsgs", "extra", "cache", "use_order", "use_limit", "static", "cur", "status")
+                 "out_extra", "fsgs", "extra", "cache", "use_order", "use_limit", "static", "cur", "status", "early")
 
     def __init__(self, device, stream, view, g, P, W, H, geom, img, radii, out_color, out_invdepth, out_extra, fsgs, extra,
                  cache, use_order, use_limit, static):
@@ -41,15 +41,19 @@
         self.out_color, self.out_invdepth, self.out_extra = out_color, out_invdepth, out_extra
         self.fsgs, self.extra = fsgs, extra
         self.cache, self.use_order, self.use_limit, self.static = cache, use_order, use_limit, static
-        self.cur = self.status = None
+        self.cur = self.status = self.early = None
 
 
 class _Last:
-    __slots__ = ("geom", "P", "view", "g", "keep", "raw", "step", "radii", "img", "done")
+    __slots__ = ("geom", "P", "view", "g", "keep", "raw", "step", "radii", "img", "done", "binning", "cap")
 
     def __init__(self, geom, P, view, g, keep, raw):
         self.geom, self.P, self.view, self.g, self.keep, self.raw = geom, P, view, g, keep, raw
-        self.step = self.radii = self.img = self.done = None
+        self.step = self.radii = self.img = self.done = self.binning = self.cap = None
+
+
+class _Early:
+    __slots__ = ("view", "g", "token", "P", "geom", "img", "binning", "cap", "radii", "limit", "limit_version", "event", "keep")
 
 
 class RasterBackend:
@@ -96,6 +100,10 @@
         self.keep_workspace = False
         self.last_workspace = None
         self._zero_images = {}
+        self.early_request = None
+        self.early_token = None
+        self._early = None
+        self.early_geometry_stats = dict(issued=0, used=0, stale=0)
 
     def _stream(self, device):
         if device.type == "cuda":
@@ -210,6 +218,7 @@
                 self._update_hint(max(st[0], st[3] * regions), limited=True)
                 self.last_deferred_num_rendered = st[0]
             if not ok:
+                self.drop_early_geometry()
                 self.depth_limit_stats["failed"] += 1
                 if st[2] != 0 or not regions:
                     d["cache"]["limit_ok"] = False
@@ -365,6 +374,78 @@
     TWO_PHASE_MIN_P = 100_000
     REACHED_SPLIT = os.environ.get("GS_REACHED_SPLIT", "1") != "0"
 
+    EARLY_GEOMETRY = os.environ.get("GS_EARLY_GEOMETRY", "1") != "0"
+
+    def request_early_geometry(self, settings, camera_key, token):
+        self.early_request = (settings, camera_key, token) if self.EARLY_GEOMETRY else None
+
+    def _retire_early(self, e):
+        self.early_geometry_stats["stale"] += 1
+        torch.cuda.current_stream(e.geom.device).wait_event(e.event)
+
+    def drop_early_geometry(self):
+        if self._early is not None:
+            self._retire_early(self._early)
+        self._early = self.early_request = None
+
+    def join_early_geometry(self):
+        if self._early is not None:
+            torch.cuda.current_stream(self._early.geom.device).wait_event(self._early.event)
+
+    def _launch_early_geometry(self, f, side):
+        req, self.early_request = self.early_request, None
+        if self._early is not None:
+            self._retire_early(self._early)
+        self._early = None
+        if (req is None or not self.EARLY_GEOMETRY or not self.REACHED_SPLIT or os.environ.get("GS_REACHED_SPLIT", "1") == "0"
+                or f.binning is None or f.view.tile_cull != 2 or not f.raw or self.static_capacity is not None
+                or self.scratch_fill is not None or self.output_fill is not None or f.step.rows_override
+                or not hasattr(self.api, "_forward_geometry_early")):
+            return
+        rs, camera_key, token = req
+        device, g = f.geom.device, f.g
+        H, W = int(rs.image_height), int(rs.image_width)
+        if (H, W) != (f.view.image_height, f.view.image_width) or g.extra_channel or g.shs_rest or g.colors_precomp or g.cov3D_precomp:
+            return
+        if any((p or 0) % 16 for p in (g.means3D, g.shs, g.opacities, g.scales, g.rotations)):
+            return
+        ws = self._rows_ws.get((device.index, self.scratch_bytes(f.P, W, H, 0)[3]))
+        if ws is None or not ws[1]:
+            return
+        c = self._cam_cache.get((device.index, W, H, ("key", camera_key)))
+        if c is None or not c["limit_ok"]:
+            return
+        e = _Early()
+        e.keep = list(f.keep)
+        e.view = self._view(e.keep, device, rs.bg, rs.viewmatrix, rs.projmatrix, rs.campos, rs.tanfovx, rs.tanfovy, H, W,
+                            rs.scale_modifier, rs.sh_degree, rs.prefiltered, rs.antialiasing, rs.debug, tile_cull=2)
+        e.g, e.token, e.P, e.geom, e.img, e.binning, e.cap, e.limit = g, token, f.P, f.geom, f.img, f.binning, f.cap, c["limit"]
+        e.limit_version = e.limit._version
+        e.radii = torch.empty((f.P,), dtype=torch.int32, device=device)
+        s = self._scratch(e.geom, e.img, e.binning, e.cap)
+        s.tile_depth_limit = e.limit.data_ptr()
+        self.api.call("forward_geometry_early", C.byref(e.view), C.byref(g), C.byref(s), e.radii.data_ptr(),
+                      C.c_void_p(side.cuda_stream))
+        e.event = torch.cuda.Event()
+        e.event.record(side)
+        self._early = e
+        self.early_geometry_stats["issued"] += 1
+
+    def _take_early_geometry(self, view, g, P, limit, request, static, fsgs, extra):
+        e, self._early = self._early, None
+        token, self.early_token = self.early_token, None
+        if e is None:
+            return None
+        hint = self._capacity_hint_limited if self._capacity_hint_limited > 0 else self._capacity_hint
+        cap = max(hint if hint > 0 else max(8 * P, 1 << 20), _regions(view.image_width, view.image_height))
+        if (self.EARLY_GEOMETRY and cap == e.cap and token is not None and token == e.token and request == "defer" and not static and not fsgs
+                and extra is None and limit is e.limit and limit._version == e.limit_version and self.fused_step is not None and self.scratch_fill is None
+                and self.output_fill is None and P == e.P and bytes(view) == bytes(e.view) and bytes(g) == bytes(e.g)
+                and self._arms_side_launch(self.fused_step, P)):
+            return e
+        self._retire_early(e)
+        return None
+
     def _two_phase(self, step, P):
         return self.TWO_PHASE and P >= self.TWO_PHASE_MIN_P and not step.grad_out[0]
 
@@ -376,6 +457,7 @@
         if f is None or f.step is None or f.done is not None:
             return False
         f.done = self._launch_uninstanced(f.geom.device, f.view, f.g, f.radii, self._scratch(f.geom, f.img), f.step)
+        self._launch_early_geometry(f, self._side_stream(f.geom.device))
         return True
 
     def _structs(self, device, bg, means3D, sh, colors_precomp, opacities, scales, rotations, cov3D_precomp, viewmatrix,
@@ -465,18 +547,23 @@
         g = self._gauss(keep, device, means3D, sh, colors_precomp, opacities, scales, rotations, cov3D_precomp, extra, raw=raw,
                         extra_gain=extra_gain, sh_rest=sh_rest)
 
-        gb, ib, _, _ = self.scratch_bytes(P, W, H, 0)
-        geom = torch.empty((gb,), **u8)
-        img = torch.empty((ib,), **u8)
-        if self.scratch_fill is not None:
-            self.scratch_fill("geom", geom)
-            self.scratch_fill("img", img)
+        early = self._take_early_geometry(view, g, P, limit, request, static, fsgs, extra) if device.type == "cuda" else None
+        if early is not None:
+            geom, img, radii = early.geom, early.img, early.radii
+        else:
+            gb, ib, _, _ = self.scratch_bytes(P, W, H, 0)
+            geom = torch.empty((gb,), **u8)
+            img = torch.empty((ib,), **u8)
+            if self.scratch_fill is not None:
+                self.scratch_fill("geom", geom)
+                self.scratch_fill("img", img)
         last = self._last = _Last(geom, P, view, g, keep, raw)
         step = self.fused_step
         if step is not None and not fsgs and device.type == "cuda" and self._arms_side_launch(step, P):
             last.step, last.radii, last.img = step, radii, img
         f = _Forward(device, self._stream(device), view, g, P, W, H, geom, img, radii, out_color, out_invdepth, out_extra, fsgs,
                      extra, cache, cache is not None and self.order_hint_on, use_limit, static)
+        f.early = early
 
         if device.type != "cuda":
             nr = (C.c_int32 * 1)()
@@ -577,10 +664,24 @@
         else:
             hint = self._capacity_hint_limited if (limited and self._capacity_hint_limited > 0) else self._capacity_hint
             cap = hint if hint > 0 else max(8 * f.P, 1 << 20)
+        early, f.early = f.early, None
+        if early is not None and (block is None or not limited or f.static):
+            self._retire_early(early)
+            early = None
         for attempt in range(6):
-            cap = max(cap, regions)
-            binning = self._new_binning(f, cap)
+            if early is not None:
+                cap, binning = early.cap, early.binning
+            else:
+                cap = max(cap, regions)
+                binning = self._new_binning(f, cap)
             s = self._scratch_of(f, binning, cap, limit)
+            if early is not None:
+                s.early_geometry_done = early.event.cuda_event
+                self._early_done = early.event
+                self.early_geometry_stats["used"] += 1
+                early = None
+            if self._last is not None and self._last.geom is f.geom:
+                self._last.binning, self._last.cap = binning, cap
             self.api.call("forward_geometry", C.byref(f.view), C.byref(f.g), C.byref(s), f.radii.data_ptr(), None, f.stream)
             if block is not None:
                 self.api.call("forward_bin", C.byref(f.view), C.byref(f.g), C.byref(s), None, f.stream)
@@ -760,6 +861,7 @@
             self._join_tile_order(device)
         arena, self.grad_arena = self.grad_arena, None
         step, self.fused_step = self.fused_step, None
+        self.early_request = None
         sh_rest, self.sh_rest = self.sh_rest, None
         sh_activated, self.sh_rest_activated = self.sh_rest_activated, False
         f = self._last if self._last is not None and self._last.geom is geomBuffer else None
diff --git a/sparse-view-3dgs-pack_amd/gsplat_amd/trainer.py b/sparse-view-3dgs-pack_amd/gsplat_amd/trainer.py
--- a/sparse-view-3dgs-pack_amd/gsplat_amd/trainer.py
+++ b/sparse-view-3dgs-pack_amd/gsplat_amd/trainer.py
@@ -1141,7 +1141,7 @@
         return (k * self.world_size + self.rank) % len(self.cameras)
 
     def step(self, k):
-        return self._step_camera(self.camera_index(k), self.optimizer_step, ())
+        return self._step_camera(self.camera_index(k), self.optimizer_step, (), next_ci=self.camera_index(k + 1))
 
     def draw_cameras(self, seed):
         import random
@@ -1256,6 +1256,9 @@
         g = getattr(self, "_graphed", None)
         if g is not None:
             g.settle()
+        be = self._backend()
+        if be is not None and hasattr(be, "join_early_geometry"):
+            be.join_early_geometry()
         p, self._pending = getattr(self, "_pending", None), None
         if p is None:
             return
@@ -1267,6 +1270,8 @@
                 return
         elif p["verdict"]():
             return
+        if be is not None and hasattr(be, "drop_early_geometry"):
+            be.drop_early_geometry()
         opt = self.model.optimizer
         opt.t, opt.seg_steps = p["counters"][0], dict(p["counters"][1])
         if p.get("exposure_steps") is not None:
@@ -1391,14 +1396,31 @@
                 and getattr(getattr(fn, "_impl", None), "backend", None) is not None
                 and type(self)._render_view is Trainer._render_view and type(self)._criterion_backward is Trainer._criterion_backward)
 
-    def _manual_step(self, ci, mask, backend, deferred):
+    def _raster_settings(self, ci):
         m, cam = self.model, self.cameras[ci]
-        fn = self.Rasterizer._fn
-        rs = self.Settings(
+        return self.Settings(
             image_height=int(cam.image_height), image_width=int(cam.image_width), tanfovx=math.tan(cam.FoVx * 0.5),
             tanfovy=math.tan(cam.FoVy * 0.5), bg=self.bg, scale_modifier=1.0, viewmatrix=cam.world_view_transform,
             projmatrix=cam.full_proj_transform, sh_degree=m.active_sh_degree, campos=cam.camera_center, prefiltered=False,
             debug=False, antialiasing=False)
+
+    def _early_token(self, ci):
+        m, cam = self.model, self.cameras[ci]
+        return (m.generation, m.P, m.active_sh_degree, id(m.optimizer), m.optimizer.t, m.flat._version,
+                tuple(p._version for p in m.params.values()),
+                tuple(t._version for t in (cam.world_view_transform, cam.full_proj_transform, cam.camera_center)))
+
+    def _early_geometry_ok(self, backend, fused_step, deferred):
+        m = self.model
+        return (fused_step and deferred and not m.with_nir and not self.RENDERS_NIR and self.world_size == 1
+                and getattr(self, "rows_override", None) is None and hasattr(backend, "request_early_geometry")
+                and backend.static_capacity is None and getattr(self, "_graphed", None) is None
+                and type(self)._render_view is Trainer._render_view)
+
+    def _manual_step(self, ci, mask, backend, deferred):
+        m = self.model
+        fn = self.Rasterizer._fn
+        rs = self._raster_settings(ci)
         backend.camera_key = ("trainer", self.uid, ci)
         backend.camera_key_limits = False
         empty = getattr(self, "_empty_cpu", None)
@@ -1487,7 +1509,7 @@
                 torch.gt(radii, 0, out=m.grad_mask.view(torch.bool))
             self.exchange_and_step(optimizer_step, skip)
 
-    def _step_camera(self, ci, optimizer_step, skip, exposure_step=None):
+    def _step_camera(self, ci, optimizer_step, skip, exposure_step=None, next_ci=None):
         self.sync()
         m = self.model
         if exposure_step is None:
@@ -1502,6 +1524,9 @@
                                and (m.exposure is not None or self.alpha_masks is not None))
         deferred = (fused_step or fused_dp) and self.depth_limit == "deferred" and getattr(self, "_coef_dev", None) is None \
             and (not self._image_extras() or stage_ok)
+        early_ok = self._early_geometry_ok(backend, fused_step, deferred)
+        if early_ok:
+            backend.early_token = self._early_token(ci)
         if deferred:
             counters = (m.optimizer.t, dict(m.optimizer.seg_steps))
             backend.depth_limit_request = "defer"
@@ -1518,6 +1543,9 @@
                 backend.fused_step.rows_override = rows.data_ptr()
             if self._use_stage and m.exposure is not None:
                 backend.fused_step.fail_flag = m.exposure_optimizer.gate.data_ptr()
+            if early_ok and next_ci is not None:
+                backend.request_early_geometry(self._raster_settings(next_ci), ("trainer", self.uid, next_ci),
+                                               self._early_token(next_ci))
         elif backend is not None and hasattr(backend, "grad_arena") and not m.with_nir:
             m.arm_grad_arena(backend)
         mask = None if self.masks is None else self.masks[ci]
```

New measurement: 1305 (median of 6 runs). +1.9%, better.
